# pola-rs/polars

Measured on AMD Instinct MI355X. Metric: rows/sec + achieved HBM GB/s, TPC-H Q1/Q3 SF100, 1/2/4/8 GPU vs CPU, higher is better.
Workload: dtype f64; 1 GPU; tpch_q1_sf100; rows_per_gpu=600000000, algorithmic_bytes_per_gpu_step=25200000000, parallelism=single GPU

## Files before the change

include/polars_amd.h:

```cpp
#ifndef POLARS_AMD_H
#define POLARS_AMD_H

#include <stddef.h>
#include <stdint.h>

#ifdef __cplusplus
extern "C" {
#endif

#define PLX_ABI_MAJOR 0
#define PLX_ABI_MINOR 1

#define PLX_OK 0
#define PLX_ERR_INVALID 1
#define PLX_ERR_HIP 2
#define PLX_ERR_UNSUPPORTED 3
#define PLX_ERR_OOM 4
#define PLX_ERR_SHAPE 5
#define PLX_ERR_NOT_FOUND 6
#define PLX_ERR_CANCELLED 7

typedef enum plx_dtype {
  PLX_BOOL = 0,
  PLX_I8 = 1,
// ... 181 lines not shown
  PLX_AE_IS_NOT_NULL = 9,
  PLX_AE_FILL_NULL = 10,
  PLX_AE_TERNARY = 11,
  PLX_AE_BITMAP_LOOKUP = 12,
  PLX_AE_TEMPORAL = 13
} plx_aexpr_kind;

typedef enum plx_operator {
  PLX_OP_EQ = 0, PLX_OP_NE = 1, PLX_OP_LT = 2, PLX_OP_LE = 3, PLX_OP_GT = 4, PLX_OP_GE = 5,
  PLX_OP_PLUS = 6, PLX_OP_MINUS = 7, PLX_OP_MULTIPLY = 8, PLX_OP_TRUE_DIVIDE = 9,
  PLX_OP_FLOOR_DIVIDE = 10, PLX_OP_MODULUS = 11, PLX_OP_AND = 12, PLX_OP_OR = 13, PLX_OP_XOR = 14
} plx_operator;

typedef struct plx_aexpr {
  int32_t kind;
  int32_t op;
  int32_t lhs;
  int32_t rhs;
  int32_t dtype;
  int32_t is_null;
  plx_scalar lit;
  const char* name;
  int32_t cond;
} plx_aexpr;

typedef enum plx_ir_kind {
  PLX_IR_SCAN = 0,
  PLX_IR_FILTER = 1,
  PLX_IR_SELECT = 2,
  PLX_IR_HSTACK = 3,
  PLX_IR_GROUPBY = 4,
  PLX_IR_JOIN = 5,
  PLX_IR_SORT = 6,
  PLX_IR_SLICE = 7
} plx_ir_kind;

typedef enum plx_join_order {
  PLX_JOIN_ORDER_NONE = 0,
  PLX_JOIN_ORDER_LEFT = 1,
  PLX_JOIN_ORDER_RIGHT = 2,
  PLX_JOIN_ORDER_LEFT_RIGHT = 3,
  PLX_JOIN_ORDER_RIGHT_LEFT = 4
} plx_join_order;

typedef struct plx_ir {
  int32_t kind;
  int32_t input;
  int32_t input_right;
  int32_t predicate;
  plx_frame frame;
  const int32_t* exprs;
  int32_t n_exprs;
  const int32_t* keys;
  int32_t n_keys;
  const int32_t* keys_right;
  int32_t n_keys_right;
  int32_t how;
  int32_t maintain_order;
  const char* suffix;
  const uint8_t* sort_descending;
  const uint8_t* sort_nulls_last;
  int64_t slice_offset;
  int64_t slice_len;
  int32_t coalesce;
} plx_ir;

#define PLX_PLAN_NO_FUSION 1u
#define PLX_PLAN_NO_PARTITION 4u
#define PLX_PLAN_NO_DIRECT_JOIN 2u

int plx_execute_plan(const plx_ir* ir, int32_t n_ir, const plx_aexpr* exprs, int32_t n_exprs, int32_t root,
                     uint32_t flags, plx_frame* out);
int plx_describe_fusion(const plx_ir* ir, int32_t n_ir, const plx_aexpr* exprs, int32_t n_exprs, int32_t root, int32_t* fusable,
                        int32_t* static_shape_id, char* why_not, size_t why_cap);
int plx_debug_program_json(const plx_ir* ir, int32_t n_ir, const plx_aexpr* exprs, int32_t n_exprs, int32_t root, char* buf, size_t cap);
int plx_jit_selftest(const plx_ir* ir, int32_t n_ir, const plx_aexpr* exprs, int32_t n_exprs, int32_t root);
int plx_jit_stats(int32_t* compiled, double* compile_ms);
int plx_jit_set_min_rows(int64_t min_rows);
const char* plx_last_plan_description(void);
const char* plx_last_plan_encodings(void);
int32_t plx_last_scan_tile_rows(void);
int32_t plx_wide_tiles_choice(int32_t compiled, int32_t knob_on, int64_t n_rows, int32_t n_inputs, const int32_t* dtypes, const int32_t* nullable, const uint64_t* values,
                              const uint64_t* validity);

int plx_datagen_lineitem_q1(int64_t n_rows, uint64_t seed, plx_column* out_cols);
int plx_datagen_lineitem_q1_host(int64_t row0, int64_t n, uint64_t seed, int64_t* shipdate, uint8_t* returnflag, uint8_t* linestatus,
                                 int64_t* quantity, double* extendedprice, double* discount, double* tax);

int plx_datagen_orders_lineitem(int64_t n_orders, uint64_t seed, plx_column* out_orders, plx_column* out_lineitem);
int plx_datagen_orders_lineitem_host(int64_t order0, int64_t n, int64_t n_orders_total, uint64_t seed, int64_t* orderkey, int64_t* custkey,
                                     int64_t* orderdate, uint32_t* n_lines, int64_t line_cap, int64_t* l_orderkey, double* l_extendedprice,
                                     double* l_discount, int64_t* l_shipdate, int64_t* n_lines_out);
int plx_datagen_customer(int64_t n_customers, uint64_t seed, plx_column* out_cols);
int plx_datagen_customer_host(int64_t row0, int64_t n, uint64_t seed, int64_t* custkey, uint8_t* segment);
int plx_datagen_uniform(int32_t dtype, int64_t n_rows, uint64_t seed, uint32_t stream, int64_t lo, int64_t hi, double scale, plx_column* out);
int plx_datagen_uniform_host(int32_t dtype, int64_t row0, int64_t n, uint64_t seed, uint32_t stream, int64_t lo, int64_t hi, double scale, void* out);
int plx_datagen_zipf(int64_t n_rows, uint64_t seed, uint32_t stream, uint64_t x0_q62, int64_t n_keys, plx_column* out);
int plx_datagen_zipf_host(int64_t row0, int64_t n, uint64_t seed, uint32_t stream, uint64_t x0_q62, int64_t n_keys, int64_t* out);

typedef uint64_t plx_strdict;
int plx_strview_dict_encode(const void* views, const uint8_t* validity, int64_t bit_offset, int64_t n, const void* const* data_buffers, const int64_t* data_sizes,
                            int32_t n_data_buffers, plx_column* out_codes, plx_strdict* out_dict);
int plx_strview_dict_encode_device(plx_column views_u64_pairs, plx_column data_u8, plx_column* out_codes, plx_strdict* out_dict);
int plx_strview_stamp_nulls(plx_column views_u64_pairs, plx_column valid_bool);
int plx_strview_groupby(plx_column views_u64_pairs, plx_column value, plx_column* out_codes, plx_strdict* out_dict, plx_column* out_sum, plx_column* out_count, plx_column* out_len);
#define PLX_STR_MATCH_MAX_PATTERN 64
typedef enum plx_str_match_kind { PLX_STR_STARTS_WITH = 0, PLX_STR_ENDS_WITH = 1, PLX_STR_CONTAINS = 2 } plx_str_match_kind;
int plx_strdict_match(plx_strdict dict, int32_t kind, const uint8_t* pattern, int64_t pattern_len, plx_column* out_bool);
int plx_strview_match(plx_column views_u64_pairs, plx_column data_u8, int32_t kind, const uint8_t* pattern, int64_t pattern_len, plx_column* out_bool);
int plx_strview_match_host(const void* views, const uint8_t* data, int64_t data_len, int64_t n, int32_t kind, const uint8_t* pattern, int64_t pattern_len,
                           uint64_t* out_bits, uint64_t* out_valid);
int plx_bitmap_lookup(plx_column codes, plx_column lut_bool, plx_column* out_bool);
int plx_strdict_info(plx_strdict dict, int64_t* n_strings, int64_t* total_bytes);

typedef enum plx_time_unit { PLX_UNIT_DATE = 0, PLX_UNIT_MS = 1, PLX_UNIT_US = 2, PLX_UNIT_NS = 3 } plx_time_unit;
typedef enum plx_temporal_part_kind {
  PLX_PART_YEAR = 0, PLX_PART_MONTH = 1, PLX_PART_DAY = 2, PLX_PART_QUARTER = 3, PLX_PART_WEEKDAY = 4, PLX_PART_ORDINAL_DAY = 5,
  PLX_PART_HOUR = 6, PLX_PART_MINUTE = 7, PLX_PART_SECOND = 8, PLX_PART_DATE = 9
} plx_temporal_part_kind;
int plx_temporal_part(plx_column col, int part, int unit, plx_column* out);
int plx_temporal_part_host(const void* values, int unit, int part, int64_t n, void* out);

int plx_strdict_to_host(plx_strdict dict, int64_t* offsets, uint8_t* bytes);
int plx_strdict_free(plx_strdict dict);
int plx_datagen_id_views(int64_t n_rows, uint64_t seed, uint32_t stream, int64_t lo, int64_t hi, plx_column* out_views);
int plx_datagen_long_id_views(int64_t n_rows, uint64_t seed, uint32_t stream, int64_t lo, int64_t hi, plx_column* out_views, plx_column* out_data);

typedef uint64_t plx_parquet;
int plx_parquet_open(const char* path, plx_parquet* out);
int plx_parquet_close(plx_parquet file);
int plx_parquet_shape(plx_parquet file, int64_t* num_rows, int32_t* num_row_groups, int32_t* num_columns);
int plx_parquet_column_info(plx_parquet file, int32_t column, const char** name, int32_t* dtype, int32_t* logical, int32_t* nullable);
int plx_parquet_column_timezone(plx_parquet file, int32_t column, const char** timezone);
int plx_parquet_row_group_info(plx_parquet file, int32_t row_group, int64_t* num_rows, int64_t* compressed_bytes);
int plx_parquet_chunk_info(plx_parquet file, int32_t row_group, int32_t column, int32_t* codec, uint32_t* encodings, int64_t* compressed_bytes,
                           int64_t* uncompressed_bytes, int32_t* has_min_max, plx_scalar* min, plx_scalar* max, int64_t* null_count);
int plx_parquet_read(plx_parquet file, const int32_t* row_groups, int32_t n_row_groups, const int32_t* columns, int32_t n_columns, plx_frame* out);
int plx_parquet_categories(plx_parquet file, int32_t column, int64_t* n_strings, int64_t* total_bytes);
int plx_parquet_categories_to_host(plx_parquet file, int32_t column, int64_t* offsets, uint8_t* bytes);
int plx_parquet_column_strdict(plx_parquet file, int32_t column, plx_strdict* out);

typedef uint64_t plx_ipc;
int plx_ipc_open(const char* path, plx_ipc* out);
int plx_ipc_close(plx_ipc file);
int plx_ipc_shape(plx_ipc file, int64_t* num_rows, int32_t* num_batches, int32_t* num_columns);
int plx_ipc_column_info(plx_ipc file, int32_t column, const char** name, int32_t* dtype, int32_t* logical, int32_t* nullable);
int plx_ipc_column_timezone(plx_ipc file, int32_t column, const char** timezone);
int plx_ipc_batch_info(plx_ipc file, int32_t batch, int64_t* num_rows, int64_t* body_bytes, int32_t* compressed);
int plx_ipc_read(plx_ipc file, const int32_t* batches, int32_t n_batches, const int32_t* columns, int32_t n_columns, plx_frame* out);
int plx_ipc_read_string_views(plx_ipc file, const int32_t* batches, int32_t n_batches, int32_t column, plx_column* out_views, plx_column* out_data);
int plx_ipc_categories(plx_ipc file, int32_t column, int64_t* n_strings, int64_t* total_bytes);
int plx_ipc_categories_to_host(plx_ipc file, int32_t column, int64_t* offsets, uint8_t* bytes);
int plx_ipc_column_strdict(plx_ipc file, int32_t column, plx_strdict* out);

typedef uint64_t plx_comm;
int plx_comm_unique_id(uint8_t* out_128_bytes);
int plx_comm_init(const uint8_t* unique_id_128_bytes, int32_t rank, int32_t world_size, plx_comm* out);
int plx_comm_info(plx_comm comm, int32_t* rank, int32_t* world_size);
int plx_comm_free(plx_comm comm);
int plx_exchange_by_key(plx_comm comm, plx_frame frame, const char* key, uint64_t seed, plx_frame* out, uint64_t* rows_sent, uint64_t* bytes_sent);
int plx_allgather_frame(plx_comm comm, plx_frame frame, plx_frame* out);

typedef struct plx_profile_record {
  char name[48];
  double start_us;
  double end_us;
// ... 33 lines not shown
```

polars_amd/_ffi.py:

```python
from __future__ import annotations

import ctypes as C
import os
import threading
from typing import Optional

os.environ.setdefault("GPU_MAX_HW_QUEUES", "8")

_HERE = os.path.dirname(os.path.abspath(__file__))
LIB_PATH = os.path.join(_HERE, "libpolars_amd.so")

BOOL, I8, I16, I32, I64, U8, U16, U32, U64, F32, F64 = range(11)
EQ, NE, LT, LE, GT, GE = range(6)
ADD, SUB, MUL, TRUE_DIV, FLOOR_DIV, MOD = range(6)
AND, OR, XOR = range(3)
AGG_SUM, AGG_MEAN, AGG_MIN, AGG_MAX, AGG_COUNT, AGG_LEN, AGG_FIRST, AGG_VAR, AGG_STD = range(9)
AGG_QUANTILE = 9
QUANTILE_NEAREST, QUANTILE_LOWER, QUANTILE_HIGHER, QUANTILE_MIDPOINT, QUANTILE_LINEAR = range(5)
QUANTILE_INTERPOLATIONS = {"nearest": QUANTILE_NEAREST, "lower": QUANTILE_LOWER, "higher": QUANTILE_HIGHER, "midpoint": QUANTILE_MIDPOINT, "linear": QUANTILE_LINEAR}
JOIN_INNER, JOIN_LEFT, JOIN_SEMI, JOIN_ANTI, JOIN_FULL, JOIN_RIGHT = range(6)
JOIN_COALESCE_DEFAULT, JOIN_COALESCE, JOIN_KEEP_BOTH = range(3)
JOIN_ORDER_NONE, JOIN_ORDER_LEFT, JOIN_ORDER_RIGHT, JOIN_ORDER_LEFT_RIGHT, JOIN_ORDER_RIGHT_LEFT = range(5)
AE_COLUMN, AE_LITERAL, AE_BINARY, AE_CAST, AE_AGG, AE_LEN, AE_ALIAS, AE_NOT, AE_IS_NULL, AE_IS_NOT_NULL, AE_FILL_NULL, AE_TERNARY, AE_BITMAP_LOOKUP, AE_TEMPORAL = range(14)
STR_STARTS_WITH, STR_ENDS_WITH, STR_CONTAINS = range(3)
# ... 120 lines not shown
    "plx_parquet_shape": (C.c_int, [C.c_uint64, _i64p, _i32p, _i32p]),
    "plx_parquet_column_info": (C.c_int, [C.c_uint64, C.c_int32, C.POINTER(C.c_char_p), _i32p, _i32p, _i32p]),
    "plx_parquet_column_timezone": (C.c_int, [C.c_uint64, C.c_int32, C.POINTER(C.c_char_p)]),
    "plx_parquet_row_group_info": (C.c_int, [C.c_uint64, C.c_int32, _i64p, _i64p]),
    "plx_parquet_chunk_info": (C.c_int, [C.c_uint64, C.c_int32, C.c_int32, _i32p, C.POINTER(C.c_uint32), _i64p, _i64p, _i32p, C.POINTER(Scalar), C.POINTER(Scalar), _i64p]),
    "plx_parquet_read": (C.c_int, [C.c_uint64, _i32p, C.c_int32, _i32p, C.c_int32, _u64p]),
    "plx_parquet_categories": (C.c_int, [C.c_uint64, C.c_int32, _i64p, _i64p]),
    "plx_parquet_categories_to_host": (C.c_int, [C.c_uint64, C.c_int32, C.c_void_p, C.c_void_p]),
    "plx_parquet_column_strdict": (C.c_int, [C.c_uint64, C.c_int32, _u64p]),
    "plx_ipc_open": (C.c_int, [C.c_char_p, _u64p]),
    "plx_ipc_close": (C.c_int, [C.c_uint64]),
    "plx_ipc_shape": (C.c_int, [C.c_uint64, _i64p, _i32p, _i32p]),
    "plx_ipc_column_info": (C.c_int, [C.c_uint64, C.c_int32, C.POINTER(C.c_char_p), _i32p, _i32p, _i32p]),
    "plx_ipc_column_timezone": (C.c_int, [C.c_uint64, C.c_int32, C.POINTER(C.c_char_p)]),
    "plx_ipc_batch_info": (C.c_int, [C.c_uint64, C.c_int32, _i64p, _i64p, _i32p]),
    "plx_ipc_read": (C.c_int, [C.c_uint64, _i32p, C.c_int32, _i32p, C.c_int32, _u64p]),
    "plx_ipc_read_string_views": (C.c_int, [C.c_uint64, _i32p, C.c_int32, C.c_int32, _u64p, _u64p]),
    "plx_ipc_categories": (C.c_int, [C.c_uint64, C.c_int32, _i64p, _i64p]),
    "plx_ipc_categories_to_host": (C.c_int, [C.c_uint64, C.c_int32, C.c_void_p, C.c_void_p]),
    "plx_ipc_column_strdict": (C.c_int, [C.c_uint64, C.c_int32, _u64p]),
    "plx_comm_unique_id": (C.c_int, [C.c_void_p]),
    "plx_comm_init": (C.c_int, [C.c_void_p, C.c_int32, C.c_int32, _u64p]),
    "plx_comm_info": (C.c_int, [C.c_uint64, C.POINTER(C.c_int32), C.POINTER(C.c_int32)]),
    "plx_comm_free": (C.c_int, [C.c_uint64]),
    "plx_exchange_by_key": (C.c_int, [C.c_uint64, C.c_uint64, C.c_char_p, C.c_uint64, _u64p, _u64p, _u64p]),
    "plx_allgather_frame": (C.c_int, [C.c_uint64, C.c_uint64, _u64p]),
    "plx_column_import_arrow": (C.c_int, [C.POINTER(ArrowArray), C.POINTER(ArrowSchema), _u64p]),
    "plx_column_import_series": (C.c_int, [C.POINTER(SeriesExport), _u64p]),
    "plx_column_export_arrow": (C.c_int, [C.c_uint64, C.POINTER(ArrowArray), C.POINTER(ArrowSchema)]),
    "plx_column_export_series": (C.c_int, [C.c_uint64, C.c_char_p, C.POINTER(SeriesExport)]),
    "plx_column_to_host": (C.c_int, [C.c_uint64, C.c_void_p, C.c_void_p, _i32p]),
    "plx_column_copy_to_device": (C.c_int, [C.c_uint64, C.c_void_p, C.c_void_p]),
    "plx_column_info": (C.c_int, [C.c_uint64, _i32p, _i64p, _i64p]),
    "plx_column_device_ptrs": (C.c_int, [C.c_uint64, C.POINTER(C.c_void_p), C.POINTER(C.c_void_p)]),
    "plx_column_retain": (C.c_int, [C.c_uint64]),
    "plx_column_free": (C.c_int, [C.c_uint64]),
    "plx_cmp": (C.c_int, [C.c_int, C.c_uint64, C.c_uint64, _u64p]),
    "plx_cmp_scalar": (C.c_int, [C.c_int, C.c_uint64, Scalar, _u64p]),
    "plx_bitmap_binop": (C.c_int, [C.c_int, C.c_uint64, C.c_uint64, _u64p]),
    "plx_bitmap_not": (C.c_int, [C.c_uint64, _u64p]),
    "plx_arith": (C.c_int, [C.c_int, C.c_uint64, C.c_uint64, _u64p]),
    "plx_arith_scalar": (C.c_int, [C.c_int, C.c_uint64, Scalar, C.c_int, _u64p]),
    "plx_cast": (C.c_int, [C.c_uint64, C.c_int, _u64p]),
    "plx_if_then_else": (C.c_int, [C.c_uint64, C.c_uint64, C.c_uint64, _u64p]),
    "plx_filter": (C.c_int, [C.c_uint64, C.c_uint64, _u64p]),
    "plx_gather": (C.c_int, [C.c_uint64, C.c_uint64, _u64p]),
    "plx_reduce": (C.c_int, [C.c_int, C.c_uint64, C.POINTER(Scalar), _i32p, _i32p]),
    "plx_reduce_var": (C.c_int, [C.c_uint64, C.c_int32, C.c_int32, C.POINTER(Scalar), _i32p, _i32p]),
    "plx_groupby_agg": (C.c_int, [_u64p, C.c_int32, _u64p, _i32p, C.c_int32, C.c_int32, _u64p, _u64p]),
    "plx_groupby_agg_ddof": (C.c_int, [_u64p, C.c_int32, _u64p, _i32p, C.c_int32, C.c_int32, _i32p, _u64p, _u64p]),
    "plx_reduce_quantile": (C.c_int, [C.c_uint64, C.c_double, C.c_int32, C.POINTER(Scalar), _i32p, _i32p]),
    "plx_groupby_agg_params": (C.c_int, [_u64p, C.c_int32, _u64p, _i32p, C.c_int32, C.c_int32, _i32p, C.POINTER(C.c_double), _i32p, _u64p, _u64p]),
    "plx_join_indices": (C.c_int, [C.c_int, C.c_uint64, C.c_uint64, _u64p, _u64p]),
    "plx_datagen_lineitem_q1": (C.c_int, [C.c_int64, C.c_uint64, _u64p]),
    "plx_datagen_lineitem_q1_host": (C.c_int, [C.c_int64, C.c_int64, C.c_uint64, C.c_void_p, C.c_void_p, C.c_void_p, C.c_void_p, C.c_void_p, C.c_void_p, C.c_void_p]),
    "plx_datagen_orders_lineitem": (C.c_int, [C.c_int64, C.c_uint64, _u64p, _u64p]),
    "plx_datagen_orders_lineitem_host": (C.c_int, [C.c_int64, C.c_int64, C.c_int64, C.c_uint64, C.c_void_p, C.c_void_p, C.c_void_p, C.c_void_p, C.c_int64,
                                                   C.c_void_p, C.c_void_p, C.c_void_p, C.c_void_p, _i64p]),
    "plx_datagen_uniform": (C.c_int, [C.c_int32, C.c_int64, C.c_uint64, C.c_uint32, C.c_int64, C.c_int64, C.c_double, _u64p]),
    "plx_datagen_customer": (C.c_int, [C.c_int64, C.c_uint64, _u64p]),
    "plx_datagen_customer_host": (C.c_int, [C.c_int64, C.c_int64, C.c_uint64, C.c_void_p, C.c_void_p]),
    "plx_datagen_uniform_host": (C.c_int, [C.c_int32, C.c_int64, C.c_int64, C.c_uint64, C.c_uint32, C.c_int64, C.c_int64, C.c_double, C.c_void_p]),
    "plx_datagen_zipf": (C.c_int, [C.c_int64, C.c_uint64, C.c_uint32, C.c_uint64, C.c_int64, _u64p]),
    "plx_datagen_zipf_host": (C.c_int, [C.c_int64, C.c_int64, C.c_uint64, C.c_uint32, C.c_uint64, C.c_int64, C.c_void_p]),
    "plx_debug_program_json": (C.c_int, [C.POINTER(IR), C.c_int32, C.POINTER(AExpr), C.c_int32, C.c_int32, C.c_char_p, C.c_size_t]),
    "plx_sort_indices": (C.c_int, [_u64p, C.c_int32, C.POINTER(C.c_uint8), C.POINTER(C.c_uint8), C.c_int64, _u64p]),
    "plx_hash_partition": (C.c_int, [C.c_uint64, C.c_int32, C.c_uint64, _u64p, _i64p]),
    "plx_frame_new": (C.c_int, [C.POINTER(C.c_char_p), _u64p, C.c_int32, _u64p]),
    "plx_frame_free": (C.c_int, [C.c_uint64]),
    "plx_frame_concat": (C.c_int, [_u64p, C.c_int32, _u64p]),
    "plx_frame_shape": (C.c_int, [C.c_uint64, _i64p, _i32p]),
    "plx_frame_column": (C.c_int, [C.c_uint64, C.c_int32, C.POINTER(C.c_char_p), _u64p]),
    "plx_frame_dtypes": (C.c_int, [C.c_uint64, _i32p]),
    "plx_frame_to_host": (C.c_int, [C.c_uint64, C.POINTER(C.c_void_p), C.POINTER(C.c_void_p), _i32p]),
    "plx_execute_plan": (C.c_int, [C.POINTER(IR), C.c_int32, C.POINTER(AExpr), C.c_int32, C.c_int32, C.c_uint32, _u64p]),
    "plx_describe_fusion": (C.c_int, [C.POINTER(IR), C.c_int32, C.POINTER(AExpr), C.c_int32, C.c_int32, _i32p, _i32p, C.c_char_p, C.c_size_t]),
    "plx_jit_selftest": (C.c_int, [C.POINTER(IR), C.c_int32, C.POINTER(AExpr), C.c_int32, C.c_int32]),
    "plx_jit_stats": (C.c_int, [_i32p, C.POINTER(C.c_double)]),
    "plx_jit_set_min_rows": (C.c_int, [C.c_int64]),
    "plx_last_plan_description": (C.c_char_p, []),
    "plx_last_plan_encodings": (C.c_char_p, []),
    "plx_last_scan_tile_rows": (C.c_int32, []),
    "plx_wide_tiles_choice": (C.c_int32, [C.c_int32, C.c_int32, C.c_int64, C.c_int32, C.POINTER(C.c_int32), C.POINTER(C.c_int32), C.POINTER(C.c_uint64), C.POINTER(C.c_uint64)]),
    "plx_profile_enable": (C.c_int, [C.c_int]),
    "plx_profile_fetch": (C.c_int, [C.POINTER(ProfileRecord), C.c_int32, _i32p]),
    "plx_profile_clear": (C.c_int, []),
}

_lib: Optional[C.CDLL] = None


def lib() -> C.CDLL:
    global _lib
    if _lib is None:
        if not os.path.exists(LIB_PATH):
            raise ImportError(
                f"{LIB_PATH} is missing: build the HIP extension first "
                "(python -c 'import __graft_entry__ as g; g.build()' or make -C polars_amd/csrc). "
                "There is no CPU fallback in polars_amd.")
        l = C.CDLL(LIB_PATH, mode=C.RTLD_GLOBAL)
        for name, (res, args) in SIGNATURES.items():
            fn = getattr(l, name)
            fn.restype = res
            fn.argtypes = args
        _lib = l
    return _lib


def check(status: int) -> None:
    if status != 0:
        msg = lib().plx_last_error().decode("utf-8", "replace")
        if status == ERR_UNSUPPORTED:
            raise UnsupportedError(status, msg)
        raise PlxError(status, msg)


_initialised = False


def init(device: Optional[int] = None) -> None:
    global _initialised
    if device is None:
        device = int(os.environ.get("LOCAL_RANK", "0"))
    check(lib().plx_init(device))
    _initialised = True


def ensure_init() -> None:
    if not _initialised:
        init()


_tls = threading.local()


def set_plan_note(note) -> None:
    _tls.plan_note = note


def last_plan() -> str:
    note = getattr(_tls, "plan_note", None)
    return note if note is not None else lib().plx_last_plan_description().decode()


def last_plan_encodings() -> str:
    return lib().plx_last_plan_encodings().decode()


def last_scan_tile_rows() -> int:
    return int(lib().plx_last_scan_tile_rows())


def wide_tiles_choice(compiled, knob_on, n_rows, dtypes, nullable, values, validity) -> int:
    n = len(dtypes)
    return int(lib().plx_wide_tiles_choice(int(bool(compiled)), int(bool(knob_on)), int(n_rows), n, (C.c_int32 * n)(*[int(d) for d in dtypes]),
                                           (C.c_int32 * n)(*[int(bool(x)) for x in nullable]), (C.c_uint64 * n)(*[int(v) for v in values]), (C.c_uint64 * n)(*[int(v) for v in validity])))


def jit_set_min_rows(min_rows: int) -> None:
    check(lib().plx_jit_set_min_rows(int(min_rows)))


def encoded_set_decimal_min_rows(min_rows: int) -> None:
    check(lib().plx_encoded_set_decimal_min_rows(int(min_rows)))


def encoded_decimal_min_rows() -> int:
    return int(lib().plx_encoded_decimal_min_rows())


def jit_stats():
    n, ms = C.c_int32(), C.c_double()
    check(lib().plx_jit_stats(C.byref(n), C.byref(ms)))
    return n.value, ms.value
```

polars_amd/csrc/abi.cpp:

```cpp
#include <cstdio>
#include <cstring>
#include <memory>
#include <mutex>

#include "core.hpp"
#include "datagen_device.hpp"
#include "encoded_inputs.hpp"
#include "engine.hpp"
#include "fused_shapes.hpp"
#include "jit.hpp"
#include "join.hpp"
#include "kernels.hpp"
#include "kernels_fused.hpp"
#include "ops.hpp"
#include "scan.hpp"
#include "sort.hpp"
#include "strmatch.hpp"
#include "temporal.hpp"

namespace plx {
void init_device(int ordinal);
void clear_handles();
const std::string& last_error_ref();
namespace comm {
void unique_id(uint8_t* out128);
uint64_t init(const uint8_t* id128, int rank, int ws);
void destroy(uint64_t h);
void info(uint64_t h, int* rank, int* ws);
FramePtr exchange_by_key(uint64_t h, const FramePtr& in, const std::string& key, uint64_t seed, uint64_t* rows_sent, uint64_t* bytes_sent);
FramePtr allgather_frame(uint64_t h, const FramePtr& in);
}
}

using namespace plx;

#define PLX_TRY try {
#define PLX_CATCH                                                                   \
  }                                                                                 \
  catch (const plx::Error& e) { plx::set_last_error(e.msg); return e.code; }        \
  catch (const std::bad_alloc&) { plx::set_last_error("host out of memory"); return PLX_ERR_OOM; } \
  catch (const std::exception& e) { plx::set_last_error(std::string("PANIC: ") + e.what()); return PLX_ERR_INVALID; } \
  catch (...) { plx::set_last_error("PANIC"); return PLX_ERR_INVALID; }              \
  return PLX_OK;

static thread_local std::string t_plan_desc;
static thread_local std::string t_plan_encoded;

extern "C" {

uint32_t plx_version(void) { return ((uint32_t)PLX_ABI_MAJOR << 16) | (uint32_t)PLX_ABI_MINOR; }
const char* plx_last_error(void) { return plx::last_error_ref().c_str(); }

int plx_init(int device_ordinal) { PLX_TRY init_device(device_ordinal); PLX_CATCH }
int plx_shutdown(void) {
  PLX_TRY
  clear_handles();
  pool_trim();
  PLX_CATCH
}
int plx_set_stream(void* hip_stream) { PLX_TRY device(); set_thread_stream((hipStream_t)hip_stream); PLX_CATCH }
int plx_synchronize(void) { PLX_TRY PLX_HIP(hipStreamSynchronize(stream())); PLX_CATCH }
int plx_set_cancel(int flag) { PLX_TRY device().cancel.store(flag); PLX_CATCH }
int plx_device_info(char* name_out, size_t name_cap, int32_t* cu_count, uint64_t* hbm_bytes) {
  PLX_TRY
  Device& d = device();
  if (name_out && name_cap) snprintf(name_out, name_cap, "%s", d.name.c_str());
  if (cu_count) *cu_count = d.cu_count;
  if (hbm_bytes) *hbm_bytes = d.hbm_bytes;
  PLX_CATCH
}
int plx_memory_stats(uint64_t* in_use, uint64_t* high_water) { PLX_TRY pool_stats(in_use, high_water); PLX_CATCH }
int plx_memory_trim(void) { PLX_TRY pool_trim(); PLX_CATCH }
int plx_memory_reserve(uint64_t bytes) { PLX_TRY device(); pool_reserve((size_t)bytes); PLX_CATCH }

int plx_column_from_host(plx_dtype dtype, const void* values, const uint8_t* validity, int64_t bit_offset, int64_t len, plx_column* out) {
  PLX_TRY
  PLX_REQUIRE(out, PLX_ERR_INVALID, "null out pointer");
  PLX_REQUIRE(values || len == 0, PLX_ERR_INVALID, "null values pointer");
  *out = register_column(column_from_host(dtype, values, validity, bit_offset, len));
  PLX_CATCH
}
int plx_column_from_device(plx_dtype dtype, void* dev_values, void* dev_validity, int64_t len, plx_column* out) {
  PLX_TRY
  device();
  PLX_REQUIRE(out && (dev_values || len == 0), PLX_ERR_INVALID, "null pointer");
  PLX_REQUIRE(dtype >= PLX_BOOL && dtype <= PLX_F64 && len >= 0, PLX_ERR_INVALID, "column_from_device: bad dtype or length");
  const uintptr_t value_align = dtype == PLX_BOOL ? 8 : (uintptr_t)dtype_width(dtype);
  PLX_REQUIRE(((uintptr_t)dev_values % value_align) == 0, PLX_ERR_INVALID,
              std::string("column_from_device: the values pointer of a ") + dtype_name(dtype) + " column must be a multiple of " + std::to_string(value_align));
  PLX_REQUIRE(((uintptr_t)dev_validity % 8) == 0, PLX_ERR_INVALID, "column_from_device: the validity pointer must be a multiple of 8 (validity is read as 64-bit words)");
  auto c = std::make_shared<Column>();
// ... 821 lines not shown
  }
  if (n_lines_out) *n_lines_out = at;
  PLX_CATCH
}
int plx_datagen_customer(int64_t n_customers, uint64_t seed, plx_column* out_cols) {
  PLX_TRY
  PLX_REQUIRE(n_customers >= 0 && out_cols, PLX_ERR_INVALID, "datagen: bad arguments");
  ColumnPtr k = make_column(PLX_I64, n_customers, false), sgm = make_column(PLX_U8, n_customers, false);
  k->null_count = 0; sgm->null_count = 0;
  k::datagen_customer(n_customers, seed, k->values->as<int64_t>(), sgm->values->as<uint8_t>());
  out_cols[0] = register_column(k); out_cols[1] = register_column(sgm);
  PLX_CATCH
}
int plx_datagen_customer_host(int64_t row0, int64_t n, uint64_t seed, int64_t* custkey, uint8_t* segment) {
  PLX_TRY
  PLX_REQUIRE(row0 >= 0 && n >= 0, PLX_ERR_INVALID, "datagen: bad arguments");
  for (int64_t j = 0; j < n; j++) {
    if (custkey) custkey[j] = row0 + j + 1;
    if (segment) segment[j] = datagen::customer_segment(seed, (uint64_t)(row0 + j + 1));
  }
  PLX_CATCH
}
int plx_datagen_uniform(int32_t dtype, int64_t n_rows, uint64_t seed, uint32_t stream_id, int64_t lo, int64_t hi, double scale, plx_column* out) {
  PLX_TRY
  PLX_REQUIRE(n_rows >= 0 && out && hi > lo && stream_id < 8, PLX_ERR_INVALID, "datagen: bad arguments");
  PLX_REQUIRE(dtype == PLX_I64 || dtype == PLX_U32 || dtype == PLX_F64, PLX_ERR_UNSUPPORTED, "datagen_uniform: dtype must be Int64, UInt32 or Float64");
  ColumnPtr c = make_column(dtype, n_rows, false); c->null_count = 0;
  k::datagen_uniform(dtype, n_rows, seed, stream_id, lo, hi, scale, c->values->ptr);
  *out = register_column(c);
  PLX_CATCH
}
int plx_datagen_uniform_host(int32_t dtype, int64_t row0, int64_t n, uint64_t seed, uint32_t stream_id, int64_t lo, int64_t hi, double scale, void* out) {
  PLX_TRY
  PLX_REQUIRE(row0 >= 0 && n >= 0 && (out || n == 0) && hi > lo && stream_id < 8, PLX_ERR_INVALID, "datagen: bad arguments");
  PLX_REQUIRE(dtype == PLX_I64 || dtype == PLX_U32 || dtype == PLX_F64, PLX_ERR_UNSUPPORTED, "datagen_uniform: dtype must be Int64, UInt32 or Float64");
  for (int64_t j = 0; j < n; j++) {
    const int64_t v = datagen::uniform_value(seed, stream_id, (uint64_t)(row0 + j), lo, hi);
    if (dtype == PLX_I64) reinterpret_cast<int64_t*>(out)[j] = v;
    else if (dtype == PLX_U32) reinterpret_cast<uint32_t*>(out)[j] = (uint32_t)v;
    else reinterpret_cast<double*>(out)[j] = (double)v * scale;
  }
  PLX_CATCH
}

int plx_datagen_zipf(int64_t n_rows, uint64_t seed, uint32_t stream_id, uint64_t x0_q62, int64_t n_keys, plx_column* out) {
  PLX_TRY
  PLX_REQUIRE(n_rows >= 0 && out && n_keys > 0 && stream_id < 8 && x0_q62 > 0 && x0_q62 < (1ull << 62), PLX_ERR_INVALID, "datagen_zipf: bad arguments");
  ColumnPtr c = make_column(PLX_I64, n_rows, false); c->null_count = 0;
  k::datagen_zipf(n_rows, seed, stream_id, x0_q62, n_keys, c->values->as<int64_t>());
  *out = register_column(c);
  PLX_CATCH
}
int plx_datagen_zipf_host(int64_t row0, int64_t n, uint64_t seed, uint32_t stream_id, uint64_t x0_q62, int64_t n_keys, int64_t* out) {
  PLX_TRY
  PLX_REQUIRE(row0 >= 0 && n >= 0 && (out || n == 0) && n_keys > 0 && stream_id < 8 && x0_q62 > 0 && x0_q62 < (1ull << 62), PLX_ERR_INVALID, "datagen_zipf: bad arguments");
  for (int64_t j = 0; j < n; j++) out[j] = datagen::zipf_value(seed, stream_id, (uint64_t)(row0 + j), x0_q62, n_keys);
  PLX_CATCH
}

int plx_execute_plan(const plx_ir* ir, int32_t n_ir, const plx_aexpr* exprs, int32_t n_exprs, int32_t root, uint32_t flags, plx_frame* out) {
  PLX_TRY
  PLX_REQUIRE(out, PLX_ERR_INVALID, "null out pointer");
  engine::Plan p = engine::import_plan(ir, n_ir, exprs, n_exprs, flags);
  FramePtr f = engine::execute(p, root);
  t_plan_desc = p.desc;
  t_plan_encoded = p.encoded;
  *out = register_frame(f);
  PLX_CATCH
}
const char* plx_last_plan_description(void) { return t_plan_desc.c_str(); }
const char* plx_last_plan_encodings(void) { return t_plan_encoded.c_str(); }
int32_t plx_last_scan_tile_rows(void) { return k::last_scan_tile_rows(); }
int32_t plx_wide_tiles_choice(int32_t compiled, int32_t knob_on, int64_t n_rows, int32_t n_inputs, const int32_t* dtypes, const int32_t* nullable, const uint64_t* values,
                              const uint64_t* validity) {
  if (n_inputs < 0 || n_inputs > fused::kMaxInputs || (n_inputs && (!dtypes || !nullable || !values || !validity))) return -1;
  fused::Shape sh{}; fused::Args args{};
  sh.n_inputs = (uint8_t)n_inputs; sh.pred = fused::kNone; sh.key = fused::kNone;
  args.n_rows = n_rows;
  for (int i = 0; i < n_inputs; i++) {
    sh.in_dtype[i] = (uint8_t)dtypes[i]; sh.in_nullable[i] = (uint8_t)(nullable[i] != 0);
    args.in[i].values = (const void*)(uintptr_t)values[i]; args.in[i].validity = (const uint64_t*)(uintptr_t)validity[i];
  }
  return k::wide_tiles_choice(sh, args, compiled != 0, knob_on != 0) ? 1 : 0;
}

int plx_debug_program_json(const plx_ir* ir, int32_t n_ir, const plx_aexpr* exprs, int32_t n_exprs, int32_t root, char* buf, size_t cap) {
  PLX_TRY
  PLX_REQUIRE(buf && cap > 0, PLX_ERR_INVALID, "null buffer");
  engine::Plan p = engine::import_plan(ir, n_ir, exprs, n_exprs, 0);
  std::string json, why;
  if (!engine::dump_program_json(p, root, &json, &why)) fail(PLX_ERR_UNSUPPORTED, "not a fusable pipeline: " + why);
  PLX_REQUIRE(json.size() + 1 <= cap, PLX_ERR_INVALID, "buffer too small for the program dump (" + std::to_string(json.size() + 1) + " bytes)");
  memcpy(buf, json.c_str(), json.size() + 1);
  PLX_CATCH
}

int plx_describe_fusion(const plx_ir* ir, int32_t n_ir, const plx_aexpr* exprs, int32_t n_exprs, int32_t root, int32_t* fusable, int32_t* static_shape_id,
                        char* why_not, size_t why_cap) {
  PLX_TRY
  engine::Plan p = engine::import_plan(ir, n_ir, exprs, n_exprs, 0);
  auto dump = [](const fused::Shape& sh) {
    std::string d = "inputs=" + std::to_string(sh.n_inputs) + " pred=" + std::to_string(sh.pred) + " key=" + std::to_string(sh.key) + " ops=[";
    for (int i = 0; i < sh.n_ops; i++) d += "(" + std::to_string(sh.ops[i].code) + "," + std::to_string(sh.ops[i].dst) + "," + std::to_string(sh.ops[i].a) + "," + std::to_string(sh.ops[i].b) + "," + std::to_string(sh.ops[i].c) + ")";
    d += "] aggs=[";
    for (int i = 0; i < sh.n_aggs; i++) d += "(" + std::to_string(sh.aggs[i].kind) + "," + std::to_string(sh.aggs[i].src) + ")";
    d += "] in_dtype=[";
    for (int i = 0; i < sh.n_inputs; i++) d += std::to_string(sh.in_dtype[i]) + (sh.in_nullable[i] ? "?" : "") + ",";
    d += "]";
    if (sh.n_keys) { d += " keys=["; for (int i = 0; i < sh.n_keys; i++) d += std::to_string(sh.keys[i]) + ","; d += "]"; }
    return d;
  };
  std::string why;
  int sid = -1;
  bool ok;
  PLX_REQUIRE(root >= 0 && root < (int)p.ir.size(), PLX_ERR_INVALID, "bad root");
  const engine::IRN& rn = p.ir[root];
  if (rn.kind == PLX_IR_GROUPBY && rn.input >= 0 && p.ir[rn.input].kind == PLX_IR_JOIN) {
    std::vector<fused::Shape> shapes;
    ok = engine::describe_join_fusion(p, root, &shapes, &why);
    if (ok) {
      sid = fused::find_static_shape(shapes[2]);
      t_plan_desc = dump(shapes[0]);
      for (size_t i = 1; i < shapes.size(); i++) t_plan_desc += "\n" + dump(shapes[i]);
    }
  } else {
    fused::Shape sh{};
    ok = engine::describe_fusion(p, root, &sh, &sid, &why);
    if (ok) t_plan_desc = dump(sh);
  }
  if (fusable) *fusable = ok ? 1 : 0;
  if (static_shape_id) *static_shape_id = sid;
  if (why_not && why_cap) snprintf(why_not, why_cap, "%s", why.c_str());
  PLX_CATCH
}

int plx_jit_selftest(const plx_ir* ir, int32_t n_ir, const plx_aexpr* exprs, int32_t n_exprs, int32_t root) {
  PLX_TRY
  engine::Plan p = engine::import_plan(ir, n_ir, exprs, n_exprs, 0);
  PLX_REQUIRE(root >= 0 && root < (int)p.ir.size(), PLX_ERR_INVALID, "bad root");
  const engine::IRN& rn = p.ir[root];
  std::string why;
  std::vector<std::pair<fused::Shape, jit::Sink>> jobs;
  if (rn.kind == PLX_IR_GROUPBY && rn.input >= 0 && p.ir[rn.input].kind == PLX_IR_JOIN) {
    std::vector<fused::Shape> shapes;
    PLX_REQUIRE(engine::describe_join_fusion(p, root, &shapes, &why), PLX_ERR_UNSUPPORTED, "not fusable: " + why);
    jobs = {{shapes[0], jit::REGAGG}, {shapes[1], jit::JOIN_BUILD}, {shapes[1], jit::DIRECT_BUILD}, {shapes[2], jit::PROBE_AGG}, {shapes[2], jit::DIRECT_PROBE}};
    for (size_t i = 3; i + 1 < shapes.size(); i++) jobs.push_back({shapes[i], jit::BITMAP_BUILD});
    for (uint32_t tiles : {2u, 4u}) jobs.push_back({shapes.back(), jit::part3_scatter_sink(fused::kP2Direct, tiles, fused::kPackRowid, false)});
  } else if (rn.kind == PLX_IR_FILTER) {
    fused::Shape sh{};
    PLX_REQUIRE(engine::describe_filter_fusion(p, root, &sh, &why), PLX_ERR_UNSUPPORTED, "not fusable: " + why);
    jobs = {{sh, jit::BALLOT}};
  } else {
    fused::Shape sh{}; int sid = -1;
    PLX_REQUIRE(engine::describe_fusion(p, root, &sh, &sid, &why), PLX_ERR_UNSUPPORTED, "not fusable: " + why);
    if (rn.kind == PLX_IR_SELECT) jobs = {{sh, jit::REGAGG}};
    else jobs = {{sh, jit::LDSAGG}, {sh, jit::DENSE}, {sh, jit::HASH}, {sh, jit::PART_COUNT}, {sh, jit::PART_SCATTER}, {sh, jit::PART_AGG},
                  {sh, jit::PART2_SCATTER_HASH}, {sh, jit::PART2_SCATTER_DIRECT}, {sh, jit::PART2_AGG_HASH}, {sh, jit::PART2_AGG_DIRECT},
                  {sh, jit::PART2_SCATTER_HASH_T2}, {sh, jit::PART2_SCATTER_DIRECT_T2}};
    if (rn.kind != PLX_IR_SELECT && sh.n_keys < 2) {
      for (uint32_t mode = 0; mode < 2; mode++) {
        const uint32_t best = fused::best_static_pack(sh, mode);
        for (uint32_t pack = 0; pack <= best; pack++) {
          if (pack == fused::kPackNarrow && fused::rec_layout2(sh, mode, fused::kPackNarrow).rec_words == fused::rec_layout2(sh, mode, fused::kPackNone).rec_words) continue;
          for (uint32_t tiles : {1u, 2u, 3u, 4u}) { jobs.push_back({sh, jit::part3_scatter_sink(mode, tiles, pack, false)}); jobs.push_back({sh, jit::part3_scatter_sink(mode, tiles, pack, true)}); }
          jobs.push_back({sh, jit::part3_agg_sink(mode, pack)});
        }
      }
      for (uint32_t mode = 0; mode < 2; mode++) {
        if (!fused::pair_pack_ok(sh, mode)) continue;
        for (uint32_t tiles : {1u, 2u, 3u, 4u}) { if (mode == fused::kP2Hash && tiles > 3) continue; jobs.push_back({sh, jit::part3_scatter_sink(mode, tiles, fused::kPackPair, false)}); jobs.push_back({sh, jit::part3_scatter_sink(mode, tiles, fused::kPackPair, true)}); }
        jobs.push_back({sh, jit::part3_agg_sink(mode, fused::kPackPair)});
      }
      if (fused::pairv_pack_ok(sh, fused::kP2Hash)) {
        for (uint32_t tiles : {1u, 2u, 3u}) { jobs.push_back({sh, jit::part3_scatter_sink(fused::kP2Hash, tiles, fused::kPackPairV, false)}); jobs.push_back({sh, jit::part3_scatter_sink(fused::kP2Hash, tiles, fused::kPackPairV, true)}); }
        jobs.push_back({sh, jit::part3_agg_sink(fused::kP2Hash, fused::kPackPairV)});
      }
    }
    if (sh.n_keys >= 2) {
      jobs = {{sh, jit::WIDE}};
      for (uint32_t pack = 0; pack <= std::min<uint32_t>(fused::best_static_pack(sh, fused::kP2Hash), fused::kPackNarrow); pack++) {
        for (uint32_t tiles : {1u, 2u, 3u}) jobs.push_back({sh, jit::part3_scatter_sink(fused::kP2Hash, tiles, pack, false)});
        jobs.push_back({sh, jit::part3_agg_sink(fused::kP2Hash, pack)});
      }
    }
  }
  {
    std::vector<std::pair<fused::Shape, jit::Sink>> forms;
    fused::Args aligned{}; aligned.n_rows = fused::kWideTileRows;
    for (auto& j : jobs) {
      const bool wide = k::wide_tiles_choice(j.first, aligned, true, true);
      if (j.second == jit::REGAGG && wide) forms.push_back({j.first, jit::REGAGG_WIDE});
      if (j.second == jit::LDSAGG && wide) forms.push_back({j.first, jit::LDSAGG_WIDE});
    }
    jobs.insert(jobs.end(), forms.begin(), forms.end());
  }
  for (auto& j : jobs) {
    const std::string log = jit::selftest(j.first, j.second);
    if (!log.empty()) fail(PLX_ERR_INVALID, "jit selftest failed: " + log.substr(0, 4000));
  }
  PLX_CATCH
}
int plx_jit_set_min_rows(int64_t min_rows) { PLX_TRY jit::set_min_rows(min_rows); PLX_CATCH }
int plx_jit_stats(int32_t* compiled, double* compile_ms) {
  PLX_TRY
  int c = 0; double ms = 0;
  jit::stats(&c, &ms);
  if (compiled) *compiled = c;
  if (compile_ms) *compile_ms = ms;
  PLX_CATCH
}

extern "C++" {
namespace {
struct StrDict { Buf views, data, offsets, bytes; int64_t n = 0; uint64_t total = 0; bool materialised = false; };
std::mutex g_strdict_mu;
std::vector<std::unique_ptr<StrDict>> g_strdicts;
StrDict& get_strdict(uint64_t h) {
  std::lock_guard<std::mutex> lk(g_strdict_mu);
  if (h == 0 || h > g_strdicts.size() || !g_strdicts[h - 1]) fail(PLX_ERR_INVALID, "invalid string dictionary handle");
  return *g_strdicts[h - 1];
}
uint64_t register_strdict(std::unique_ptr<StrDict> d) { std::lock_guard<std::mutex> lk(g_strdict_mu); g_strdicts.push_back(std::move(d)); return (uint64_t)g_strdicts.size(); }
void materialise(StrDict& d) {
  if (d.materialised) return;
  k::strdict_materialise(d.views->as<uint64_t>(), d.data ? d.data->as<uint8_t>() : nullptr, d.n, &d.offsets, &d.bytes, &d.total);
  d.materialised = true;
}
void encode_on_device(const uint64_t* views, const ColumnPtr& validity_holder, Buf data, Buf buf_base, int64_t n, plx_column* out_codes, plx_strdict* out_dict, bool from_stamps = false) {
  Buf codes, dviews, svalid;
  int64_t nd = 0, snulls = 0;
  k::strview_dict_encode(views, validity_holder ? validity_holder->valid_words() : nullptr, data ? data->as<uint8_t>() : nullptr, buf_base ? buf_base->as<uint64_t>() : nullptr, n, &codes, &dviews, &nd,
                         from_stamps && !validity_holder ? &svalid : nullptr, &snulls);
  auto c = std::make_shared<Column>();
  c->dtype = PLX_U32; c->len = n; c->values = codes;
  if (validity_holder && validity_holder->validity) c->validity = validity_holder->validity;
  else if (snulls > 0) { c->validity = svalid; c->null_count = snulls; }
  else c->null_count = 0;
  if (nd > 0) { c->range_state = 1; c->range_min = 0; c->range_max = nd - 1; c->range_trusted = true; }
  auto d = std::make_unique<StrDict>();
  d->views = dviews; d->data = data; d->n = nd;
  *out_codes = register_column(c);
  *out_dict = register_strdict(std::move(d));
}
}
namespace plx {
void strview_encode_device(const uint64_t* views, const ColumnPtr& validity_holder, Buf data, int64_t n, plx_column* out_codes, plx_strdict* out_dict) {
  Buf bb = dev_alloc_zero(8);
  encode_on_device(views, validity_holder, data, bb, n, out_codes, out_dict);
}
void strview_encode_device_bases(const uint64_t* views, const ColumnPtr& validity_holder, Buf data, Buf buf_base, int64_t n, plx_column* out_codes, plx_strdict* out_dict) {
  encode_on_device(views, validity_holder, data, buf_base, n, out_codes, out_dict);
}
}
}

int plx_strview_dict_encode(const void* views, const uint8_t* validity, int64_t bit_offset, int64_t n, const void* const* data_buffers, const int64_t* data_sizes,
                            int32_t n_data_buffers, plx_column* out_codes, plx_strdict* out_dict) {
  PLX_TRY
  PLX_REQUIRE(out_codes && out_dict && n >= 0 && (views || n == 0) && n_data_buffers >= 0 && (n_data_buffers == 0 || (data_buffers && data_sizes)), PLX_ERR_INVALID, "strview_dict_encode: bad arguments");
  device();
  Buf dv = dev_alloc((size_t)std::max<int64_t>(n, 1) * 16);
  if (n) h2d_sync_pinned(dv->ptr, views, (size_t)n * 16);
  ColumnPtr vh;
  if (validity) {
    std::vector<uint8_t> zeros((size_t)n);
    vh = column_from_host(PLX_U8, zeros.data(), validity, bit_offset, n);
  }
  uint64_t total = 0;
  std::vector<uint64_t> base((size_t)std::max(n_data_buffers, 1), 0);
  for (int i = 0; i < n_data_buffers; i++) { base[i] = total; total += (uint64_t)data_sizes[i]; }
  Buf data = dev_alloc((size_t)total + 64), bb = dev_alloc(sizeof(uint64_t) * base.size());
  for (int i = 0; i < n_data_buffers; i++) {
    if (!data_sizes[i]) continue;
    if ((uint64_t)data_sizes[i] >= ((uint64_t)32 << 20)) h2d_sync_pinned((uint8_t*)data->ptr + base[i], data_buffers[i], (size_t)data_sizes[i]);
    else h2d_async((uint8_t*)data->ptr + base[i], data_buffers[i], (size_t)data_sizes[i]);
// ... 248 lines not shown
```

polars_amd/csrc/fused_device.hpp:

```cpp
#pragma once
#include "decimal.hpp"
#include "dev.hpp"
#include "fused.hpp"
#include "fused_shapes.hpp"
#include "kconfig.hpp"
#include "temporal.hpp"

namespace plx {
namespace k {

using namespace dev;
using namespace fused;

typedef unsigned long long u64x16 __attribute__((ext_vector_type(16)));
typedef unsigned int u32x16 __attribute__((ext_vector_type(16)));

struct RegFile {
  uint64_t v[kRows][kSlots];
  uint32_t valid[kSlots];
  __device__ __forceinline__ uint64_t get(int r, int s) const { return v[r][s]; }
  __device__ __forceinline__ uint32_t getv(int s) const { return valid[s]; }
  __device__ __forceinline__ void set(int r, int s, uint64_t x) { v[r][s] = x; }
  __device__ __forceinline__ void setv(int s, uint32_t m) { valid[s] = m; }
};
struct LdsRegFile {
  unsigned long long* vals;
  unsigned int* vbits;
  int lane;
  __device__ __forceinline__ uint64_t get(int r, int s) const { return vals[(s * kRows + r) * 64 + lane]; }
  __device__ __forceinline__ uint32_t getv(int s) const { return vbits[s * 64 + lane]; }
  __device__ __forceinline__ void set(int r, int s, uint64_t x) { vals[(s * kRows + r) * 64 + lane] = x; }
  __device__ __forceinline__ void setv(int s, uint32_t m) { vbits[s * 64 + lane] = m; }
};
__host__ __device__ constexpr unsigned lds_regfile_bytes_per_wave(unsigned slots) { return slots * (kRows * 64 * 8 + 64 * 4); }

__device__ __forceinline__ int dtype_width_dev(int dt) {
  switch (dt) {
    case PLX_I8: case PLX_U8: return 1;
    case PLX_I16: case PLX_U16: return 2;
    case PLX_I32: case PLX_U32: case PLX_F32: return 4;
    default: return 8;
  }
}
__device__ __forceinline__ double as_f(uint64_t x) { return __longlong_as_double((long long)x); }
__device__ __forceinline__ uint64_t as_u(double x) { return (uint64_t)__double_as_longlong(x); }

template <class T, bool FULL>
__device__ __forceinline__ void load2(const void* base_ptr, int64_t row0, int64_t n, uint64_t out[kRows]) {
  const T* p = reinterpret_cast<const T*>(base_ptr);
  if constexpr (FULL) {
    Pack<T, kRows> x = load_pack<T, kRows>(p + row0);
#pragma unroll
    for (int r = 0; r < kRows; r++) {
      if constexpr (is_fp<T>::value) out[r] = as_u((double)x.v[r]);
      else out[r] = (uint64_t)(long long)x.v[r];
    }
  } else {
#pragma unroll
    for (int r = 0; r < kRows; r++) {
      int64_t i = row0 + r; if (i > n - 1) i = n - 1;
      T x = p[i];
      if constexpr (is_fp<T>::value) out[r] = as_u((double)x);
      else out[r] = (uint64_t)(long long)x;
    }
  }
}

template <bool FULL>
__device__ __forceinline__ void load_input(const Input& in, int dtype, int64_t row0, int64_t n, uint64_t out[kRows], uint32_t& vbits, bool may_be_null = true) {
  switch (dtype) {
    case PLX_I64: case PLX_U64: case PLX_F64: load2<uint64_t, FULL>(in.values, row0, n, out); break;
    case PLX_I32: load2<int32_t, FULL>(in.values, row0, n, out); break;
    case PLX_U32: load2<uint32_t, FULL>(in.values, row0, n, out); break;
    case PLX_I16: load2<int16_t, FULL>(in.values, row0, n, out); break;
    case PLX_U16: load2<uint16_t, FULL>(in.values, row0, n, out); break;
    case PLX_I8: load2<int8_t, FULL>(in.values, row0, n, out); break;
    case PLX_U8: load2<uint8_t, FULL>(in.values, row0, n, out); break;
    case PLX_BOOL: {
      int64_t i = row0; if (!FULL && i > n - 1) i = n - 1;
      uint64_t w = reinterpret_cast<const uint64_t*>(in.values)[i >> 6] >> (i & 63);
      out[0] = w & 1; out[1] = (w >> 1) & 1;
    } break;
    default: out[0] = out[1] = 0; break;
  }
  vbits = (1u << kRows) - 1;
  if (may_be_null && in.validity) {
// ... 290 lines not shown
    for (int pc = 0; pc < sh.n_ops; pc++) exec_op<FULL, ND, TRUST_NULLABLE>(sh.ops[pc], sh, args, pc, row0, rf);
  } else {
    Prefetched pf;
    pf.bits0 = 0; pf.bits1 = 0; pf.vword = 0;
    prefetch_inputs<FULL>(dsh, args, row0, pf);
    store_prefetched<FULL>(dsh, args, row0, pf, rf);
    const int first = dsh.n_inputs < kPrefetch ? dsh.n_inputs : kPrefetch;
    for (int pc = first; pc < dsh.n_ops; pc++) exec_op<FULL>(dsh.ops[pc], dsh, args, pc, row0, rf);
  }
}

__host__ __device__ constexpr int leading_loads(const Shape& s) {
  int n = 0;
  while (n < s.n_ops && s.ops[n].code == OP_LOAD) n++;
  return n;
}
__host__ __device__ constexpr int shape_row_bytes(const Shape& s) {
  int b = 0;
  for (int i = 0; i < s.n_inputs; i++) {
    switch (s.in_dtype[i]) {
      case PLX_I8: case PLX_U8: b += 1; break;
      case PLX_I16: case PLX_U16: b += 2; break;
      case PLX_I32: case PLX_U32: case PLX_F32: b += 4; break;
      case PLX_BOOL: break;
      default: b += 8; break;
    }
  }
  return b;
}
__host__ __device__ constexpr bool narrow_rows(const Shape& s) { return s.n_inputs > 0 && shape_row_bytes(s) <= 16; }
__host__ __device__ constexpr int wide_dtype_bytes(int dt) {
  switch (dt) {
    case PLX_I8: case PLX_U8: return 1;
    case PLX_I16: case PLX_U16: return 2;
    case PLX_I32: case PLX_U32: return 4;
    case PLX_I64: case PLX_U64: case PLX_F64: return 8;
    default: return 0;
  }
}
__host__ __device__ constexpr bool wide_tiles_shape(const Shape& s) {
  if (!narrow_rows(s)) return false;
  bool any_narrow = false;
  for (int i = 0; i < s.n_inputs; i++) {
    if (s.in_nullable[i] != 0 || wide_dtype_bytes(s.in_dtype[i]) == 0) return false;
    any_narrow = any_narrow || wide_dtype_bytes(s.in_dtype[i]) < 8;
  }
  if (!any_narrow) return false;
  for (int pc = 0; pc < s.n_ops; pc++) if (s.ops[pc].code == OP_LOAD && s.ops[pc].a >= s.n_inputs) return false;
  return true;
}
struct WideRaw { uint32_t w[kMaxInputs][2 * kWideRows]; };
template <class P>
__device__ __forceinline__ void wide_load(const Args& args, int64_t row0, WideRaw& raw) {
  constexpr Shape sh = P::shape();
#pragma unroll
  for (int i = 0; i < kMaxInputs; i++) {
    if (i < sh.n_inputs) {
      const int wb = wide_dtype_bytes(sh.in_dtype[i]);
      const unsigned char* p = reinterpret_cast<const unsigned char*>(args.in[i].values) + row0 * wb;
      if (wb == 1) {
        const uint2 x = *reinterpret_cast<const uint2*>(p);
        raw.w[i][0] = x.x; raw.w[i][1] = x.y;
      } else {
#pragma unroll
        for (int q = 0; q < wb / 2; q++) {
          const uint4 x = reinterpret_cast<const uint4*>(p)[q];
          raw.w[i][4 * q] = x.x; raw.w[i][4 * q + 1] = x.y; raw.w[i][4 * q + 2] = x.z; raw.w[i][4 * q + 3] = x.w;
        }
      }
    }
  }
}
__device__ __forceinline__ uint64_t wide_unpack(const uint32_t* w, int dt, int e) {
  switch (dt) {
    case PLX_I8: return (uint64_t)(long long)(int8_t)(w[e >> 2] >> ((e & 3) * 8));
    case PLX_U8: return (uint64_t)(uint8_t)(w[e >> 2] >> ((e & 3) * 8));
    case PLX_I16: return (uint64_t)(long long)(int16_t)(w[e >> 1] >> ((e & 1) * 16));
    case PLX_U16: return (uint64_t)(uint16_t)(w[e >> 1] >> ((e & 1) * 16));
    case PLX_I32: return (uint64_t)(long long)(int32_t)w[e];
    case PLX_U32: return (uint64_t)w[e];
    default: return (uint64_t)w[2 * e] | ((uint64_t)w[2 * e + 1] << 32);
  }
}
template <class P, int ND, class RF>
__device__ __forceinline__ void run_program_wide(const Args& args, const WideRaw& raw, int j, RF& rf) {
  constexpr Shape sh = P::shape();
#pragma unroll
  for (int pc = 0; pc < sh.n_ops; pc++) {
    const Op op = sh.ops[pc];
    if (op.code == OP_LOAD) {
#pragma unroll
      for (int r = 0; r < kRows; r++) rf.set(r, op.dst, wide_unpack(raw.w[op.a], sh.in_dtype[op.a], kRows * j + r));
      rf.setv(op.dst, (1u << kRows) - 1);
    } else {
      exec_op<true, ND, true>(op, sh, args, pc, 0, rf);
    }
  }
}

template <class P, class RF>
__device__ __forceinline__ void run_loads_full(const Args& args, int64_t row0, RF& rf) {
  constexpr Shape sh = P::shape();
  constexpr int nl = leading_loads(sh);
#pragma unroll
  for (int pc = 0; pc < nl; pc++) exec_op<true>(sh.ops[pc], sh, args, pc, row0, rf);
}
template <class P, class RF>
__device__ __forceinline__ void run_rest_full(const Args& args, int64_t row0, RF& rf) {
  constexpr Shape sh = P::shape();
  constexpr int nl = leading_loads(sh);
#pragma unroll
  for (int pc = nl; pc < sh.n_ops; pc++) exec_op<true>(sh.ops[pc], sh, args, pc, row0, rf);
}

template <class P, bool FULL, bool EARLY, class RF>
__device__ __forceinline__ void run_split(const Args& args, int64_t row0, RF& rf) {
  constexpr Shape sh = P::shape();
  constexpr ProgramSplit sp = split_program(sh);
#pragma unroll
  for (int pc = 0; pc < sh.n_ops; pc++)
    if (((sp.early >> pc) & 1u) == (EARLY ? 1u : 0u)) exec_op<FULL>(sh.ops[pc], sh, args, pc, row0, rf);
}

template <class P> struct RegFileOf { using type = RegFile; };
template <> struct RegFileOf<DynProg> { using type = LdsRegFile; };
template <class P>
__device__ __forceinline__ typename RegFileOf<P>::type make_regfile(const Args& args) {
  if constexpr (P::kStatic) { return RegFile{}; }
  else {
    extern __shared__ unsigned long long plx_dyn_lds[];
    const unsigned per_wave = lds_regfile_bytes_per_wave(args.rf_slots);
    unsigned char* base = reinterpret_cast<unsigned char*>(plx_dyn_lds) + args.rf_lds_offset + (threadIdx.x >> 6) * per_wave;
    LdsRegFile rf;
    rf.vals = reinterpret_cast<unsigned long long*>(base);
    rf.vbits = reinterpret_cast<unsigned int*>(base + (size_t)args.rf_slots * kRows * 64 * 8);
    rf.lane = lane_id();
    return rf;
  }
}

__device__ __forceinline__ uint64_t agg_combine(uint8_t kind, uint64_t x, uint64_t y) {
  switch (kind) {
    case AGG_SUM_F: return as_u(as_f(x) + as_f(y));
    case AGG_MIN_F: return as_u(min_ign<double>(as_f(x), as_f(y)));
    case AGG_MAX_F: return as_u(max_ign<double>(as_f(x), as_f(y)));
    case AGG_MIN_I: return (uint64_t)((long long)x < (long long)y ? (long long)x : (long long)y);
    case AGG_MAX_I: return (uint64_t)((long long)x > (long long)y ? (long long)x : (long long)y);
    case AGG_MIN_U: case AGG_FIRST_ROW: return x < y ? x : y;
    case AGG_MAX_U: return x > y ? x : y;
    default: return x + y;
  }
}
__device__ __forceinline__ uint64_t agg_identity_dev(uint8_t kind) {
  switch (kind) {
    case AGG_MIN_F: return 0x7ff0000000000000ull;
    case AGG_MAX_F: return 0xfff0000000000000ull;
    case AGG_MIN_I: return 0x7fffffffffffffffull;
    case AGG_MAX_I: return 0x8000000000000000ull;
    case AGG_MIN_U: case AGG_FIRST_ROW: return ~0ull;
    default: return 0ull;
  }
}
__device__ __forceinline__ uint64_t agg_row_value(uint8_t kind, uint64_t v, bool pass, bool valid, uint64_t row) {
  switch (kind) {
    case AGG_LEN: return pass ? 1ull : 0ull;
    case AGG_COUNT: return (pass && valid) ? 1ull : 0ull;
    case AGG_COUNT_ORD: { double f = as_f(v); return (pass && valid && f == f) ? 1ull : 0ull; }
    case AGG_FIRST_ROW: return pass ? row : ~0ull;
    case AGG_MIN_F: { double f = as_f(v); return (pass && valid && f == f) ? v : 0x7ff0000000000000ull; }
    case AGG_MAX_F: { double f = as_f(v); return (pass && valid && f == f) ? v : 0xfff0000000000000ull; }
    case AGG_SUM_F: case AGG_SUM_I: return (pass && valid) ? v : 0ull;
    default: return (pass && valid) ? v : agg_identity_dev(kind);
  }
}

// ... 90 lines not shown
```

polars_amd/csrc/fused_sinks.hpp:

```cpp
#pragma once
#include <type_traits>

#include "fused_device.hpp"

namespace plx {
namespace k {

struct RegAggSink {
  struct Params { unsigned long long* partials; };
  uint64_t acc[kMaxAggs];
  template <class S> __device__ __forceinline__ void init(const S& sh, const Params&) {
#pragma unroll
    for (int k = 0; k < kMaxAggs; k++) acc[k] = (k < sh.n_aggs) ? agg_identity_dev(sh.aggs[k].kind) : 0ull;
  }
  template <class S, class RF> __device__ __forceinline__ void consume(const S& sh, const RF& rf, const bool pass[kRows], int64_t row0, const Params&) {
#pragma unroll
    for (int r = 0; r < kRows; r++) {
#pragma unroll
      for (int k = 0; k < kMaxAggs; k++) {
        if (k < sh.n_aggs) {
          const Agg ag = sh.aggs[k];
          uint64_t v = rf.get(r, ag.src);
          bool valid = (rf.getv(ag.src) >> r) & 1;
          acc[k] = agg_combine(ag.kind, acc[k], agg_row_value(ag.kind, v, pass[r], valid, (uint64_t)(row0 + r)));
        }
      }
    }
  }
  template <class S> __device__ __forceinline__ void finish(const S& sh, const Params& p) {
    __shared__ uint64_t sh_acc[kBlock / 64][kMaxAggs];
    const int lane = lane_id(), wave = threadIdx.x >> 6;
#pragma unroll
    for (int k = 0; k < kMaxAggs; k++) {
      if (k < sh.n_aggs) {
        uint64_t x = acc[k];
#pragma unroll
        for (int m = 32; m >= 1; m >>= 1) x = agg_combine(sh.aggs[k].kind, x, shfl_xor_u64(x, m));
        if (lane == 0) sh_acc[wave][k] = x;
      }
    }
    __syncthreads();
    if ((int)threadIdx.x < sh.n_aggs) {
      const int k = threadIdx.x;
      uint64_t x = sh_acc[0][k];
      for (int w = 1; w < (int)(blockDim.x >> 6); w++) x = agg_combine(sh.aggs[k].kind, x, sh_acc[w][k]);
      p.partials[(size_t)blockIdx.x * kMaxAggs + k] = x;
    }
  }
};

struct LdsAggSink {
  struct Params {
    unsigned long long* partials;
    unsigned long long* global_acc;
    int n_groups;
    int copies;
    unsigned int* oob;
  };
  template <class S> __device__ __forceinline__ void init(const S& sh, const Params& p) {
    extern __shared__ unsigned long long lds_tbl[];
    const int cells = p.n_groups * sh.n_aggs;
    for (int i = threadIdx.x; i < cells * p.copies; i += blockDim.x) lds_tbl[i] = agg_identity_dev(sh.aggs[(i / p.copies) % sh.n_aggs].kind);
    __syncthreads();
  }
  template <class S, class RF> __device__ __forceinline__ void consume(const S& sh, const RF& rf, const bool pass[kRows], int64_t row0, const Params& p) {
    extern __shared__ unsigned long long lds_tbl[];
    const int copy = lane_id() & (p.copies - 1);
#pragma unroll
    for (int r = 0; r < kRows; r++) {
      if (!pass[r]) continue;
      const uint64_t gid64 = rf.get(r, sh.key);
      if (gid64 >= (uint64_t)p.n_groups) { if (p.oob) *p.oob = 1u; continue; }
      const uint32_t gid = (uint32_t)gid64;
      unsigned long long* cells = lds_tbl + (size_t)gid * sh.n_aggs * p.copies + copy;
#pragma unroll
      for (int k = 0; k < kMaxAggs; k++) {
        if (k < sh.n_aggs) {
          const Agg ag = sh.aggs[k];
          uint64_t v = rf.get(r, ag.src);
          bool valid = (rf.getv(ag.src) >> r) & 1;
          if ((ag.kind == AGG_SUM_F || ag.kind == AGG_SUM_I || ag.kind == AGG_COUNT) && !valid) continue;
          uint64_t x = agg_row_value(ag.kind, v, true, valid, (uint64_t)(row0 + r));
          lds_atomic_agg(ag.kind, cells + k * p.copies, x);
        }
      }
    }
  }
  template <class S> __device__ __forceinline__ void finish(const S& sh, const Params& p) {
    extern __shared__ unsigned long long lds_tbl[];
    __syncthreads();
    const int cells = p.n_groups * sh.n_aggs;
    for (int i = threadIdx.x; i < cells; i += blockDim.x) {
      const uint8_t kind = sh.aggs[i % sh.n_aggs].kind;
      uint64_t x = lds_tbl[(size_t)i * p.copies];
      for (int c = 1; c < p.copies; c++) x = agg_combine(kind, x, lds_tbl[(size_t)i * p.copies + c]);
      if (p.global_acc) { if (x != agg_identity_dev(kind) || kind == AGG_SUM_F) atomic_agg(kind, p.global_acc + i, x); }
      else p.partials[(size_t)blockIdx.x * cells + i] = x;
    }
  }
};

struct DenseAggSink {
  using Params = DenseTable;
  template <class S> __device__ __forceinline__ void init(const S&, const Params&) {}
  template <class S> __device__ __forceinline__ void finish(const S&, const Params&) {}
  template <class S, class RF> __device__ __forceinline__ void consume(const S& sh, const RF& rf, const bool pass[kRows], int64_t row0, const Params& p) {
#pragma unroll
    for (int r = 0; r < kRows; r++) {
      if (!pass[r]) continue;
      bool kvalid = (rf.getv(sh.key) >> r) & 1;
      int64_t g = kvalid ? ((int64_t)rf.get(r, sh.key) - p.key_min) : p.n_groups;
      if ((uint64_t)g > (uint64_t)p.n_groups || (kvalid && g == p.n_groups)) { if (p.oob) *p.oob = 1u; continue; }
      atomic_row(sh, rf, r, row0 + r, p.acc + (size_t)g * sh.n_aggs);
    }
  }
};

struct HashAggSink {
  using Params = HashTable;
  template <class S> __device__ __forceinline__ void init(const S&, const Params&) {}
  template <class S> __device__ __forceinline__ void finish(const S&, const Params&) {}
  __device__ __forceinline__ static int64_t find_slot(const Params& p, uint64_t key) {
    const uint64_t cap = 1ull << p.log2_cap;
    uint64_t slot = (key * 0x55fbfd6bfc5458e9ull) >> (64 - p.log2_cap);
    for (uint32_t probe = 0; probe < p.max_probe; probe++) {
      unsigned long long cur = p.keys[slot];
      if (cur == key) return (int64_t)slot;
      if (cur == kEmptyKey) {
        unsigned long long old = atomicCAS(&p.keys[slot], (unsigned long long)kEmptyKey, (unsigned long long)key);
        if (old == kEmptyKey || old == key) return (int64_t)slot;
      }
      slot = (slot + 1) & (cap - 1);
    }
    atomicExch(p.overflow, 1u);
    return -1;
  }
  static constexpr int kCombineRounds = 8;
  template <class S, class RF> __device__ __forceinline__ void consume_combined(const S& sh, const RF& rf, const bool pass[kRows], int64_t row0, const Params& p) {
    const uint64_t cap = 1ull << p.log2_cap;
    const int lane = lane_id();
#pragma unroll
    for (int r = 0; r < kRows; r++) {
      const bool kvalid = (rf.getv(sh.key) >> r) & 1;
      const uint64_t key = kvalid ? rf.get(r, sh.key) : 0ull;
      uint64_t xv[kMaxAggs];
#pragma unroll
      for (int k = 0; k < kMaxAggs; k++) {
        xv[k] = 0;
        if (k < sh.n_aggs) { const Agg ag = sh.aggs[k]; xv[k] = agg_row_value(ag.kind, rf.get(r, ag.src), true, (rf.getv(ag.src) >> r) & 1, (uint64_t)(row0 + r)); }
      }
      bool reached = false, keeps_total = false;
      uint64_t todo = ballot(pass[r]);
#pragma unroll 1
      for (int round = 0; round < kCombineRounds && todo; round++) {
        const int leader = (int)__builtin_ctzll(todo);
        const uint64_t lkey = shfl_u64(key, leader);
        const bool lvalid = __shfl((int)kvalid, leader, 64) != 0;
        const bool member = pass[r] && !reached && kvalid == lvalid && key == lkey;
        todo &= ~ballot(member);
#pragma unroll
        for (int k = 0; k < kMaxAggs; k++) {
          if (k < sh.n_aggs) {
            uint64_t x = member ? xv[k] : agg_identity_dev(sh.aggs[k].kind);
#pragma unroll
            for (int m = 32; m >= 1; m >>= 1) x = agg_combine(sh.aggs[k].kind, x, shfl_xor_u64(x, m));
            if (lane == leader) xv[k] = x;
          }
        }
        if (member) reached = true;
        if (lane == leader) keeps_total = true;
      }
      if (!pass[r] || (reached && !keeps_total)) continue;
      int64_t slot;
      if (!kvalid) { slot = (int64_t)cap; p.keys[cap] = 0; }
      else if (key == kEmptyKey) { slot = (int64_t)cap + 1; p.keys[cap + 1] = 0; }
      else slot = find_slot(p, key);
      if (slot < 0) continue;
#pragma unroll
      for (int k = 0; k < kMaxAggs; k++) {
        if (k < sh.n_aggs) {
          const uint8_t kind = sh.aggs[k].kind;
// ... 240 lines not shown
};

struct BitmapBuildSink {
  using Params = BitmapBuild;
  unsigned long long n = 0;
  template <class S> __device__ __forceinline__ void init(const S&, const Params&) { n = 0; }
  template <class S> __device__ __forceinline__ void finish(const S&, const Params& p) {
    const uint64_t w = wave_sum_u64(n);
    if (lane_id() == 0 && w) atomicAdd(p.count, (unsigned long long)w);
  }
  template <class S, class RF> __device__ __forceinline__ void consume(const S& sh, const RF& rf, const bool pass[kRows], int64_t, const Params& p) {
#pragma unroll
    for (int r = 0; r < kRows; r++) {
      if (!pass[r] || !((rf.getv(sh.key) >> r) & 1)) continue;
      const uint64_t idx = rf.get(r, sh.key) - (uint64_t)p.kmin;
      if (idx >= p.range) continue;
      n++;
      __hip_atomic_fetch_or(&p.bits[idx >> 6], 1ull << (idx & 63), __ATOMIC_RELAXED, __HIP_MEMORY_SCOPE_AGENT);
    }
  }
};

struct DirectHitsSink {
  using Params = DirectHits;
  template <class S> __device__ __forceinline__ void init(const S&, const Params&) {}
  template <class S> __device__ __forceinline__ void finish(const S&, const Params&) {}
  template <class S, class RF> __device__ __forceinline__ void consume(const S& sh, const RF& rf, const bool pass[kRows], int64_t row0, const Params& p) {
    bool hit[kRows];
#pragma unroll
    for (int r = 0; r < kRows; r++) {
      bool ok = pass[r] && ((rf.getv(sh.key) >> r) & 1);
      const uint64_t idx = rf.get(r, sh.key) - (uint64_t)p.t.kmin;
      ok = ok && idx < p.t.range;
      if (ok) ok = (p.t.bits[idx >> 6] >> (idx & 63)) & 1ull;
      hit[r] = ok;
    }
    const unsigned long long b0 = ballot(hit[0]), b1 = ballot(hit[1]);
    if (lane_id() == 0) {
      const int64_t t = row0 / kTileRows;
      *reinterpret_cast<ulonglong2*>(p.out.ballots + t * 2) = make_ulonglong2(b0, b1);
      p.out.counts[t] = (unsigned int)(popc64(b0) + popc64(b1));
    }
  }
};

template <class P, bool FULL>
__device__ __forceinline__ void direct_probe_tile(const Args& args, const DirectJoinTable& p, int64_t base, RegFile& rf) {
  constexpr Shape sh = P::shape();
  const int64_t row0 = base + (int64_t)lane_id() * kRows;
  run_split<P, FULL, true>(args, row0, rf);
  if (!(p.opts & kDirectLateLoads)) run_split<P, FULL, false>(args, row0, rf);
  bool hit[kRows], any = false;
  unsigned long long slot[kRows];
#pragma unroll
  for (int r = 0; r < kRows; r++) {
    bool ok = FULL || (row0 + r < args.n_rows);
    if (sh.pred != kNone) ok = ok && (rf.get(r, sh.pred) & 1) && ((rf.getv(sh.pred) >> r) & 1);
    ok = ok && ((rf.getv(sh.key) >> r) & 1);
    const uint64_t idx = rf.get(r, sh.key) - (uint64_t)p.kmin;
    ok = ok && idx < p.range;
    slot[r] = 0;
    if (ok) {
      const unsigned long long w = p.bits[idx >> 6];
      ok = (w >> (idx & 63)) & 1ull;
      if (ok) slot[r] = direct_slot(p, idx, w);
    }
    hit[r] = ok; any = any || ok;
  }
  if (any) {
    if (p.opts & kDirectLateLoads) run_split<P, FULL, false>(args, row0, rf);
#pragma unroll
    for (int r = 0; r < kRows; r++)
      if (hit[r]) atomic_row(sh, rf, r, row0 + r, p.acc + (size_t)slot[r] * sh.n_aggs);
  }
}

template <class P, class Sink>
__host__ __device__ constexpr bool late_probe() {
  if constexpr (P::kStatic && std::is_same<Sink, DirectProbeAggSink>::value) return split_program(P::shape()).any_late;
  else return false;
}
template <class P, class Sink>
__host__ __device__ constexpr bool trust_nullable() {
  if constexpr (P::kStatic && (std::is_same<Sink, LdsAggSink>::value || std::is_same<Sink, RegAggSink>::value)) return narrow_rows(P::shape());
  else return false;
}
template <class P, class Sink>
__host__ __device__ constexpr bool wide_tiles_form() {
  if constexpr (trust_nullable<P, Sink>()) return wide_tiles_shape(P::shape());
  else return false;
}
template <class P, class Sink, bool WIDE = false>
__device__ __forceinline__ void fused_scan_body(const Shape dsh, const Args args, const typename Sink::Params sp) {
  Sink sink;
  typename RegFileOf<P>::type rf = make_regfile<P>(args);
  const int64_t wave = ((int64_t)blockIdx.x * blockDim.x + threadIdx.x) >> 6;
  const int64_t nwaves = ((int64_t)gridDim.x * blockDim.x) >> 6;
  const int64_t ntiles = (args.n_rows + kTileRows - 1) / kTileRows;
  if constexpr (late_probe<P, Sink>()) {
    for (int64_t t = wave; t < ntiles; t += nwaves) {
      const int64_t base = t * kTileRows;
      if (base + kTileRows <= args.n_rows) direct_probe_tile<P, true>(args, sp, base, rf);
      else direct_probe_tile<P, false>(args, sp, base, rf);
    }
  } else if constexpr (P::kStatic) {
    constexpr Shape sh = P::shape();
    constexpr int ND = dict_count(sh);
    constexpr bool kTrust = trust_nullable<P, Sink>();
    if constexpr (ND > 0) { stage_dicts<ND>(args); __syncthreads(); }
    sink.init(sh, sp);
    int64_t first_tile = 0;
    if constexpr (WIDE) {
      static_assert(wide_tiles_form<P, Sink>(), "wide tiles: a compiled aggregate scan over narrow rows without nullable inputs");
      const int64_t nwide = args.n_rows / kWideTileRows;
      const int lane = lane_id();
      for (int64_t t = wave; t < nwide; t += nwaves) {
        const int64_t row0 = t * kWideTileRows + (int64_t)lane * kWideRows;
        WideRaw raw;
        wide_load<P>(args, row0, raw);
#pragma unroll
        for (int j = 0; j < kWideRows / kRows; j++) {
          run_program_wide<P, ND>(args, raw, j, rf);
          bool pass[kRows];
#pragma unroll
          for (int r = 0; r < kRows; r++) pass[r] = sh.pred == kNone || ((rf.get(r, sh.pred) & 1) && ((rf.getv(sh.pred) >> r) & 1));
          sink.consume(sh, rf, pass, row0 + kRows * j, sp);
        }
      }
      first_tile = nwide * (kWideTileRows / kTileRows);
    }
    for (int64_t t = first_tile + wave; t < ntiles; t += nwaves) {
      bool pass[kRows]; int64_t row0;
      tile_rows<P, ND, kTrust>(dsh, args, t, rf, pass, row0);
      sink.consume(sh, rf, pass, row0, sp);
    }
    sink.finish(sh, sp);
  } else {
    sink.init(dsh, sp);
    for (int64_t t = wave; t < ntiles; t += nwaves) {
      bool pass[kRows]; int64_t row0;
      tile_rows<P>(dsh, args, t, rf, pass, row0);
      sink.consume(dsh, rf, pass, row0, sp);
    }
    sink.finish(dsh, sp);
  }
}

template <class P, class Sink>
__global__ __launch_bounds__(kBlock) void fused_scan_kernel(Shape dsh, Args args, typename Sink::Params sp) {
  fused_scan_body<P, Sink>(dsh, args, sp);
}
template <class P, class Sink>
__global__ __launch_bounds__(kBlock) void fused_scan_wide_kernel(Shape dsh, Args args, typename Sink::Params sp) {
  fused_scan_body<P, Sink, true>(dsh, args, sp);
}

struct BallotSink {
  using Params = BallotOut;
  template <class S> __device__ __forceinline__ void init(const S&, const Params&) {}
  template <class S> __device__ __forceinline__ void finish(const S&, const Params&) {}
  template <class S, class RF> __device__ __forceinline__ void consume(const S&, const RF&, const bool pass[kRows], int64_t row0, const Params& p) {
    const unsigned long long b0 = ballot(pass[0]), b1 = ballot(pass[1]);
    if (lane_id() == 0) {
      const int64_t t = row0 / kTileRows;
      *reinterpret_cast<ulonglong2*>(p.ballots + t * 2) = make_ulonglong2(b0, b1);
      p.counts[t] = (unsigned int)(popc64(b0) + popc64(b1));
    }
  }
};

}
}
```

polars_amd/csrc/jit.cpp:

```cpp
#include "jit.hpp"

#include <dlfcn.h>
#include <sys/stat.h>
#include <unistd.h>
#include <hip/hip_runtime_api.h>
#include <hip/hiprtc.h>

#include <atomic>
#include <chrono>
#include <cstdlib>
#include <cstring>
#include <map>
#include <mutex>
#include <sstream>
#include <string>
#include <vector>

#include "core.hpp"
#include "kconfig.hpp"

namespace plx {
namespace jit {

using namespace fused;

namespace {
struct Entry { hipModule_t mod = nullptr; hipFunction_t fn = nullptr; bool failed = false; };
std::mutex g_mu;
std::map<std::string, Entry> g_cache;
int g_compiled = 0;
double g_ms = 0;

bool wide_tiles(Sink s) { return s == REGAGG_WIDE || s == LDSAGG_WIDE; }
const char* sink_type(Sink s) {
  static const char* n[] = {"RegAggSink", "LdsAggSink", "DenseAggSink", "HashAggSink", "WideAggSink", "JoinBuildSink", "ProbeAggSink", "DirectBuildSink", "DirectProbeAggSink", "BitmapBuildSink",
                            "part_count", "part_scatter", "part_agg", "part2_scatter_hash", "part2_scatter_direct", "part2_agg_hash", "part2_agg_direct", "part2_scatter_hash_t2", "part2_scatter_direct_t2"};
  if (s == REGAGG_WIDE) return "RegAggSink";
  if (s == LDSAGG_WIDE) return "LdsAggSink";
  if (s == PART3_AGG_PAIRV) return "part3_agg";
  if (s >= PART3_SCATTER_PAIRV && s < PART3_AGG_PAIRV) return "part3_scatter";
  if (s == PART3_AGG_PAIR || s == PART3_AGG_PAIR_DIRECT) return "part3_agg";
  if (s >= PART3_SCATTER_PAIR && s < PART3_AGG_PAIR) return "part3_scatter";
  if (s == BALLOT) return "BallotSink";
  if (s == DIRECT_HITS) return "DirectHitsSink";
  if (s >= PART3_AGG) return "part3_agg";
  if (s >= PART3_SCATTER) return "part3_scatter";
  return n[s];
}

std::string include_dir() {
  if (const char* e = getenv("PLX_JIT_INCLUDE")) return e;
  Dl_info info;
  if (dladdr((const void*)&stats, &info) && info.dli_fname) {
    std::string p = info.dli_fname;
    size_t k = p.rfind('/');
    return (k == std::string::npos ? std::string(".") : p.substr(0, k)) + "/csrc";
  }
  return "polars_amd/csrc";
}

std::string resource_include() {
  if (const char* e = getenv("PLX_JIT_CLANG_INCLUDE")) return e;
  const char* roots[] = {"/opt/rocm/lib/llvm/lib/clang", "/opt/rocm/llvm/lib/clang"};
  for (const char* r : roots) {
    for (int v = 30; v >= 14; v--) {
      const std::string p = std::string(r) + "/" + std::to_string(v) + "/include";
      if (FILE* f = fopen((p + "/stddef.h").c_str(), "r")) { fclose(f); return p; }
    }
  }
  return "/opt/rocm/lib/llvm/lib/clang/22/include";
}
std::vector<std::string> compile_options() {
  std::vector<std::string> o = {"--offload-arch=gfx950", "-O3", "-std=c++17", "-ffp-contract=off", "-munsafe-fp-atomics", "-Wno-pass-failed", "-ffreestanding",
                                "-I" + include_dir(), "-I/opt/rocm/include", "-I" + resource_include()};
  if (const char* e = getenv("PLX_JIT_DEFINES")) { std::istringstream is(e); std::string t; while (is >> t) if (t.compare(0, 2, "-D") == 0) o.push_back(t); }
  return o;
}

uint64_t fnv1a(const std::string& s, uint64_t h = 0xcbf29ce484222325ull) { for (unsigned char c : s) { h ^= c; h *= 0x100000001b3ull; } return h; }

std::string kernel_symbol(const Shape& sh, Sink sink) {
  std::string key((const char*)&sh, sizeof(Shape));
  key.push_back((char)sink);
  char out[96];
  snprintf(out, sizeof out, "plx_jit_%s_%d_%08x", sink_type(sink), (int)sink, (unsigned)(fnv1a(key) & 0xffffffffu));
  return out;
}

std::string source_for(const Shape& sh, Sink sink) {
  std::ostringstream o;
  const std::string sym = kernel_symbol(sh, sink);
  o << "#define plx_jit_kernel " << sym << "\n";
  o << ((sink == BALLOT || sink == DIRECT_HITS || wide_tiles(sink)) ? "#include \"fused_sinks.hpp\"\n" : sink >= PART3_SCATTER ? "#include \"partition3_device.hpp\"\n" : sink >= PART2_SCATTER_HASH ? "#include \"partition2_device.hpp\"\n" : sink >= PART_COUNT ? "#include \"partition_device.hpp\"\n" : "#include \"fused_sinks.hpp\"\n") << "namespace plx { namespace k {\n"
       "struct JitProg {\n  static constexpr bool kStatic = true; static constexpr int kId = -2;\n  static constexpr Shape shape() {\n    Shape s{};\n";
  o << "    s.n_inputs = " << (int)sh.n_inputs << "; s.n_ops = " << (int)sh.n_ops << "; s.n_aggs = " << (int)sh.n_aggs << "; s.pred = " << (int)sh.pred
    << "; s.key = " << (int)sh.key << "; s.n_keys = " << (int)sh.n_keys << ";\n";
  for (int i = 0; i < kMaxKeys; i++) o << "    s.keys[" << i << "] = " << (int)sh.keys[i] << ";\n";
  for (int i = 0; i < sh.n_inputs; i++) o << "    s.in_dtype[" << i << "] = " << (int)sh.in_dtype[i] << "; s.in_nullable[" << i << "] = " << (int)sh.in_nullable[i] << ";\n";
  for (int i = 0; i < sh.n_ops; i++)
    o << "    s.ops[" << i << "] = mkop(" << (int)sh.ops[i].code << ", " << (int)sh.ops[i].dst << ", " << (int)sh.ops[i].a << ", " << (int)sh.ops[i].b << ", " << (int)sh.ops[i].c << ");\n";
  for (int i = 0; i < sh.n_aggs; i++) o << "    s.aggs[" << i << "] = Agg{" << (int)sh.aggs[i].kind << ", " << (int)sh.aggs[i].src << "};\n";
  o << "    return s;\n  }\n};\n";
  switch (sink) {
    case PART_COUNT:
      o << "extern \"C\" __global__ __launch_bounds__(kBlock) void plx_jit_kernel(Shape dsh, Args args, uint32_t log2_parts, unsigned int* hist) {\n"
           "  part_count_body<JitProg>(dsh, args, log2_parts, hist);\n}\n}}\n";
      break;
    case PART_SCATTER:
      o << "extern \"C\" __global__ __launch_bounds__(kBlock) void plx_jit_kernel(Shape dsh, Args args, PartitionPlan pp, const unsigned long long* part_off, "
           "const unsigned long long* wg_prefix, unsigned long long* out) {\n  part_scatter_body<JitProg>(dsh, args, pp, part_off, wg_prefix, out);\n}\n}}\n";
      break;
    case PART_AGG:
      o << "extern \"C\" __global__ __launch_bounds__(kAggBlock) void plx_jit_kernel(Shape dsh, PartitionPlan pp, PartAggParams ap) {\n"
           "  constexpr Shape csh = JitProg::shape(); constexpr RecLayout cl = rec_layout(JitProg::shape());\n  part_agg_body(csh, cl, pp, ap);\n}\n}}\n";
      break;
    case PART2_SCATTER_HASH: case PART2_SCATTER_DIRECT: case PART2_SCATTER_HASH_T2: case PART2_SCATTER_DIRECT_T2:
      o << "extern \"C\" __global__ __launch_bounds__(kP2MaxBlock) void plx_jit_kernel(Shape dsh, Args args, PartPlan2 pp, ScatterParams2 sp) {\n"
           "  part2_scatter_body<JitProg, " << ((sink == PART2_SCATTER_DIRECT || sink == PART2_SCATTER_DIRECT_T2) ? 1 : 0) << ", "
        << ((sink == PART2_SCATTER_HASH_T2 || sink == PART2_SCATTER_DIRECT_T2) ? 2 : 1) << ">(dsh, args, pp, sp);\n}\n}}\n";
      break;
    case PART2_AGG_HASH: case PART2_AGG_DIRECT:
      o << "extern \"C\" __global__ __launch_bounds__(kP2AggBlock) void plx_jit_kernel(PartPlan2 pp, AggParams2 ap) {\n"
           "  constexpr Shape csh = JitProg::shape(); constexpr RecLayout2 cl = rec_layout2(JitProg::shape(), " << (sink == PART2_AGG_DIRECT ? 1 : 0) << "u);\n"
           "  part2_agg_body<Shape, " << (sink == PART2_AGG_DIRECT ? 1 : 0) << ", p2_agg_chunks_in_flight(cl.rec_words)>(csh, cl, pp, ap);\n}\n}}\n";
      break;
    default:
      if (wide_tiles(sink)) {
        o << "extern \"C\" __global__ __launch_bounds__(kBlock) void plx_jit_kernel(Shape dsh, Args args, " << sink_type(sink)
          << "::Params sp) {\n  fused_scan_body<JitProg, " << sink_type(sink) << ", true>(dsh, args, sp);\n}\n}}\n";
        break;
      }
      if (sink == PART3_AGG_PAIRV) {
        o << "extern \"C\" __global__ __launch_bounds__(kP2AggBlock) void plx_jit_kernel(PartPlan2 pp, AggParams2 ap) {\n"
             "  constexpr Shape csh = JitProg::shape(); constexpr RecLayout2 cl = rec_layout2(JitProg::shape(), 0u, " << fused::kPackPairV << "u);\n"
             "  part2_agg_body<Shape, 0, p2_agg_chunks_in_flight(cl.rec_words)>(csh, cl, pp, ap);\n}\n}}\n";
        break;
      }
      if (sink >= PART3_SCATTER_PAIRV && sink < PART3_AGG_PAIRV) {
        const int v = (int)sink - (int)PART3_SCATTER_PAIRV, tiles = 1 + (v & 3), hot = (v >> 2) & 1;
        o << "extern \"C\" __global__ __launch_bounds__(kP2MaxBlock) void plx_jit_kernel(Shape dsh, Args args, PartPlan2 pp, ScatterParams2 sp) {\n"
             "  part3_scatter_body<JitProg, 0, " << tiles << ", " << fused::kPackPairV << ", " << (hot ? "true" : "false") << ">(dsh, args, pp, sp);\n}\n}}\n";
        break;
      }
      if (sink == PART3_AGG_PAIR || sink == PART3_AGG_PAIR_DIRECT) {
        const int mode = sink == PART3_AGG_PAIR_DIRECT ? 1 : 0;
        o << "extern \"C\" __global__ __launch_bounds__(kP2AggBlock) void plx_jit_kernel(PartPlan2 pp, AggParams2 ap) {\n"
             "  constexpr Shape csh = JitProg::shape(); constexpr RecLayout2 cl = rec_layout2(JitProg::shape(), " << mode << "u, " << fused::kPackPair << "u);\n"
             "  part2_agg_body<Shape, " << mode << ", p2_agg_chunks_in_flight(cl.rec_words)>(csh, cl, pp, ap);\n}\n}}\n";
        break;
      }
      if (sink >= PART3_SCATTER_PAIR && sink < PART3_AGG_PAIR) {
        const int v = (int)sink - (int)PART3_SCATTER_PAIR, tiles = 1 + (v & 3), hot = (v >> 2) & 1, mode = v >> 3;
        o << "extern \"C\" __global__ __launch_bounds__(kP2MaxBlock) void plx_jit_kernel(Shape dsh, Args args, PartPlan2 pp, ScatterParams2 sp) {\n"
             "  part3_scatter_body<JitProg, " << mode << ", " << tiles << ", " << fused::kPackPair << ", " << (hot ? "true" : "false") << ">(dsh, args, pp, sp);\n}\n}}\n";
        break;
      }
      if (sink >= PART3_AGG && sink != BALLOT && sink != DIRECT_HITS) {
        const int v = (int)sink - (int)PART3_AGG, mode = v & 1, pack = v >> 1;
        o << "extern \"C\" __global__ __launch_bounds__(kP2AggBlock) void plx_jit_kernel(PartPlan2 pp, AggParams2 ap) {\n"
             "  constexpr Shape csh = JitProg::shape(); constexpr RecLayout2 cl = rec_layout2(JitProg::shape(), " << mode << "u, " << pack << "u);\n"
             "  part2_agg_body<Shape, " << mode << ", p2_agg_chunks_in_flight(cl.rec_words)>(csh, cl, pp, ap);\n}\n}}\n";
        break;
      }
      if (sink >= PART3_SCATTER && sink != BALLOT && sink != DIRECT_HITS) {
        const int v = (int)sink - (int)PART3_SCATTER, mode = v & 1, tiles = 1 + ((v >> 1) & 3), pack = (v >> 3) & 3, hot = v >> 5;
        o << "extern \"C\" __global__ __launch_bounds__(kP2MaxBlock) void plx_jit_kernel(Shape dsh, Args args, PartPlan2 pp, ScatterParams2 sp) {\n"
             "  part3_scatter_body<JitProg, " << mode << ", " << tiles << ", " << pack << ", " << (hot ? "true" : "false") << ">(dsh, args, pp, sp);\n}\n}}\n";
        break;
      }
      o << "extern \"C\" __global__ __launch_bounds__(kBlock) void plx_jit_kernel(Shape dsh, Args args, " << sink_type(sink)
        << "::Params sp) {\n  fused_scan_body<JitProg, " << sink_type(sink) << ">(dsh, args, sp);\n}\n}}\n";
      break;
  }
  return o.str();
}

std::atomic<int64_t> g_min_rows{-2};
bool enabled(int64_t n_rows) {
  int64_t m = g_min_rows.load(std::memory_order_relaxed);
  if (m == -2) {
    const char* off = getenv("PLX_JIT");
    const char* e = getenv("PLX_JIT_MIN_ROWS");
    m = (off && off[0] == '0') ? -1 : (e ? (int64_t)atoll(e) : (int64_t)1 << 22);
    g_min_rows.store(m, std::memory_order_relaxed);
  }
  return m >= 0 && n_rows >= m;
}

std::string cache_dir() {
  const char* off = getenv("PLX_JIT_CACHE");
  if (off && off[0] == '0') return "";
  if (const char* d = getenv("PLX_JIT_CACHE_DIR")) return d;
  const char* home = getenv("HOME");
  return home && *home ? std::string(home) + "/.cache/polars_amd/jit" : std::string("/tmp/polars_amd_jit");
}
std::string headers_fingerprint() {
  static const std::string fp = [] {
    uint64_t h = 0xcbf29ce484222325ull;
    for (const char* f : {"fused.hpp", "fused_device.hpp", "fused_sinks.hpp", "fused_shapes.hpp", "partition_device.hpp", "partition2_device.hpp", "partition3_device.hpp", "dev.hpp", "kconfig.hpp", "temporal.hpp", "decimal.hpp"}) {
      if (FILE* fp2 = fopen((include_dir() + "/" + f).c_str(), "rb")) {
        char buf[65536]; size_t n;
        while ((n = fread(buf, 1, sizeof buf, fp2)) > 0) h = fnv1a(std::string(buf, n), h);
        fclose(fp2);
      }
    }
    char out[32]; snprintf(out, sizeof out, "%016llx", (unsigned long long)h);
    return std::string(out);
  }();
  return fp;
}
std::string cache_path(const std::string& src) {
  const std::string dir = cache_dir();
  if (dir.empty()) return "";
  std::string key = src + "|" + headers_fingerprint();
  for (auto& o : compile_options()) if (o.compare(0, 2, "-I") != 0) key += "|" + o;
  char name[64]; snprintf(name, sizeof name, "/%016llx%016llx.hsaco", (unsigned long long)fnv1a(key), (unsigned long long)fnv1a(key, 0x9e3779b97f4a7c15ull));
  return dir + name;
}
bool load_cached(const std::string& path, std::vector<char>* code) {
  if (path.empty()) return false;
  FILE* f = fopen(path.c_str(), "rb");
  if (!f) return false;
  fseek(f, 0, SEEK_END); const long n = ftell(f); fseek(f, 0, SEEK_SET);
  bool ok = n > 0;
  if (ok) { code->resize((size_t)n); ok = fread(code->data(), 1, (size_t)n, f) == (size_t)n; }
  fclose(f);
  return ok;
}
void store_cached(const std::string& path, const std::vector<char>& code) {
  if (path.empty()) return;
  const std::string dir = path.substr(0, path.rfind('/'));
  std::string acc;
  for (size_t i = 1; i <= dir.size(); i++) if (i == dir.size() || dir[i] == '/') { acc = dir.substr(0, i); (void)mkdir(acc.c_str(), 0755); }
  const std::string tmp = path + ".tmp" + std::to_string((long)getpid());
  if (FILE* f = fopen(tmp.c_str(), "wb")) {
    const bool ok = fwrite(code.data(), 1, code.size(), f) == code.size();
    fclose(f);
    if (!ok || rename(tmp.c_str(), path.c_str()) != 0) (void)remove(tmp.c_str());
  }
}
int g_cache_hits = 0;

Entry compile(const Shape& sh, Sink sink) {
  Entry e;
  const auto t0 = std::chrono::steady_clock::now();
  const std::string src = source_for(sh, sink);
  const std::string cpath = cache_path(src);
  {
    std::vector<char> cached;
    if (load_cached(cpath, &cached) && hipModuleLoadData(&e.mod, cached.data()) == hipSuccess && hipModuleGetFunction(&e.fn, e.mod, kernel_symbol(sh, sink).c_str()) == hipSuccess) {
      g_cache_hits++; g_compiled++;
      if (getenv("PLX_JIT_VERBOSE")) fprintf(stderr, "[plx jit] %s: loaded from %s\n", sink_type(sink), cpath.c_str());
      return e;
    }
    (void)hipGetLastError();
    e = Entry{};
  }
  hiprtcProgram prog = nullptr;
  if (hiprtcCreateProgram(&prog, src.c_str(), "plx_jit.hip", 0, nullptr, nullptr) != HIPRTC_SUCCESS) { e.failed = true; return e; }
  const std::vector<std::string> optv = compile_options();
  std::vector<const char*> opts;
  for (auto& x : optv) opts.push_back(x.c_str());
  const hiprtcResult rc = hiprtcCompileProgram(prog, (int)opts.size(), opts.data());
  if (rc != HIPRTC_SUCCESS) {
    size_t n = 0; hiprtcGetProgramLogSize(prog, &n);
    std::string log(n, 0); if (n) hiprtcGetProgramLog(prog, &log[0]);
    set_last_error("jit: hiprtc compile failed: " + log.substr(0, 2000));
    if (getenv("PLX_JIT_VERBOSE")) fprintf(stderr, "[plx jit] compile failed:\n%s\n", log.c_str());
    hiprtcDestroyProgram(&prog);
    e.failed = true;
    return e;
  }
  size_t cs = 0; hiprtcGetCodeSize(prog, &cs);
  std::vector<char> code(cs);
  hiprtcGetCode(prog, code.data());
  hiprtcDestroyProgram(&prog);
  if (hipModuleLoadData(&e.mod, code.data()) != hipSuccess || hipModuleGetFunction(&e.fn, e.mod, kernel_symbol(sh, sink).c_str()) != hipSuccess) { e.failed = true; return e; }
  const double ms = std::chrono::duration<double, std::milli>(std::chrono::steady_clock::now() - t0).count();
  g_compiled++; g_ms += ms;
  if (getenv("PLX_JIT_VERBOSE")) fprintf(stderr, "[plx jit] %s: %.0f ms, %zu bytes\n", sink_type(sink), ms, cs);
  return e;
}
}

std::string selftest(const Shape& sh, Sink sink) {
  const std::string src = source_for(sh, sink);
  hiprtcProgram prog = nullptr;
  if (hiprtcCreateProgram(&prog, src.c_str(), "plx_jit.hip", 0, nullptr, nullptr) != HIPRTC_SUCCESS) return "hiprtcCreateProgram failed";
  const std::vector<std::string> optv = compile_options();
  std::vector<const char*> opts;
  for (auto& x : optv) opts.push_back(x.c_str());
  const hiprtcResult rc = hiprtcCompileProgram(prog, (int)opts.size(), opts.data());
  std::string log;
  if (rc != HIPRTC_SUCCESS) { size_t n = 0; hiprtcGetProgramLogSize(prog, &n); log.assign(n, 0); if (n) hiprtcGetProgramLog(prog, &log[0]); if (log.empty()) log = "hiprtc error"; }
  else if (const char* dir = getenv("PLX_JIT_DUMP_DIR")) {
    size_t cs = 0; hiprtcGetCodeSize(prog, &cs);
    std::vector<char> code(cs);
    hiprtcGetCode(prog, code.data());
    const std::string base = std::string(dir) + "/" + sink_type(sink) + (wide_tiles(sink) ? "_wide" : "") + "_" + std::to_string((int)sink);
    if (FILE* f = fopen((base + ".hsaco").c_str(), "wb")) { fwrite(code.data(), 1, code.size(), f); fclose(f); }
    if (FILE* f = fopen((base + ".hip").c_str(), "wb")) { fwrite(src.data(), 1, src.size(), f); fclose(f); }
  }
  hiprtcDestroyProgram(&prog);
  return log;
}

const char* program_mode(int static_id, int64_t n_rows) { return static_id >= 0 ? "aot" : (enabled(n_rows) ? "jit" : "generic"); }

void set_min_rows(int64_t min_rows) { g_min_rows.store(min_rows < 0 ? -1 : min_rows, std::memory_order_relaxed); }

void stats(int* compiled, double* compile_ms) {
  std::lock_guard<std::mutex> lk(g_mu);
  if (compiled) *compiled = g_compiled;
  if (compile_ms) *compile_ms = g_ms;
}

static hipFunction_t get_fn(const Shape& sh, Sink sink) {
  std::string key((const char*)&sh, sizeof(Shape));
  key.push_back((char)sink);
  std::lock_guard<std::mutex> lk(g_mu);
  auto it = g_cache.find(key);
  if (it == g_cache.end()) it = g_cache.emplace(key, compile(sh, sink)).first;
  return it->second.failed ? nullptr : it->second.fn;
}

bool ensure(const Shape& sh, Sink kind, int64_t n_rows) { return enabled(n_rows) && get_fn(sh, kind) != nullptr; }

bool launch_raw(const Shape& sh, Sink kind, void** kargs, int grid, int block, size_t lds_bytes) {
  hipFunction_t fn = get_fn(sh, kind);
  if (!fn) return false;
  const hipError_t rc = hipModuleLaunchKernel(fn, (unsigned)grid, 1, 1, (unsigned)block, 1, 1, (unsigned)lds_bytes, stream(), kargs, nullptr);
  if (rc != hipSuccess) { set_last_error(std::string("jit: launch failed: ") + hipGetErrorString(rc)); return false; }
  return true;
}

bool launch(const Shape& sh, const Args& args, Sink sink, const void* params, int grid, size_t lds_bytes) {
  if (!enabled(args.n_rows)) return false;
  Shape shc = sh; Args ac = args;
  void* kargs[] = {(void*)&shc, (void*)&ac, const_cast<void*>(params)};
  return launch_raw(sh, sink, kargs, grid, k::kBlock, lds_bytes);
}

}
}
```

polars_amd/csrc/jit.hpp:

```cpp
#pragma once
#include <cstddef>
#include <cstdint>
#include <string>

#include "fused.hpp"

namespace plx {
namespace jit {

enum Sink { REGAGG = 0, LDSAGG, DENSE, HASH, WIDE, JOIN_BUILD, PROBE_AGG, DIRECT_BUILD, DIRECT_PROBE, BITMAP_BUILD,
            PART_COUNT, PART_SCATTER, PART_AGG,
            PART2_SCATTER_HASH, PART2_SCATTER_DIRECT, PART2_AGG_HASH, PART2_AGG_DIRECT,
            PART2_SCATTER_HASH_T2, PART2_SCATTER_DIRECT_T2,
            PART3_SCATTER, PART3_AGG = PART3_SCATTER + 64,
            BALLOT = PART3_AGG + 8,
            DIRECT_HITS,
            PART3_SCATTER_PAIR, PART3_AGG_PAIR = PART3_SCATTER_PAIR + 16, PART3_AGG_PAIR_DIRECT,
            PART3_SCATTER_PAIRV, PART3_AGG_PAIRV = PART3_SCATTER_PAIRV + 8,
            REGAGG_WIDE, LDSAGG_WIDE,
            kNumSinks };
inline Sink part3_scatter_sink(uint32_t mode, uint32_t tiles, uint32_t pack, bool hot) {
  if (pack == fused::kPackPairV) return (Sink)(PART3_SCATTER_PAIRV + (tiles - 1) + (hot ? 4 : 0));
  if (pack == fused::kPackPair) return (Sink)(PART3_SCATTER_PAIR + (tiles - 1) + (hot ? 4 : 0) + 8 * mode);
  return (Sink)(PART3_SCATTER + mode + 2 * (tiles - 1) + 8 * pack + (hot ? 32 : 0));
}
inline Sink part3_agg_sink(uint32_t mode, uint32_t pack) { return pack == fused::kPackPairV ? PART3_AGG_PAIRV : pack == fused::kPackPair ? (Sink)(PART3_AGG_PAIR + mode) : (Sink)(PART3_AGG + mode + 2 * pack); }

bool launch(const fused::Shape& sh, const fused::Args& args, Sink sink, const void* params, int grid, size_t lds_bytes);
bool ensure(const fused::Shape& sh, Sink kind, int64_t n_rows);
bool launch_raw(const fused::Shape& sh, Sink kind, void** kargs, int grid, int block, size_t lds_bytes);
std::string selftest(const fused::Shape& sh, Sink sink);
const char* program_mode(int static_id, int64_t n_rows);
void set_min_rows(int64_t min_rows);
void stats(int* compiled, double* compile_ms);

}
}
```

polars_amd/csrc/kernels_fused.hip:

```cpp
#include "fused_sinks.hpp"
#include "kernels.hpp"
#include "kernels_fused.hpp"
#include "variance.hpp"
#include "scan.hpp"
#include "jit.hpp"
#include <atomic>
#include <cstring>
#include <vector>

#ifdef PLX_HAVE_Q3_SHAPES
#define PLX_STATIC_JOIN_BUILD_CASES \
  case SHAPE_Q3_BUILD: hipLaunchKernelGGL((fused_scan_kernel<StatProg<SHAPE_Q3_BUILD>, JoinBuildSink>), dim3(grid), dim3(kBlock), 0, stream(), sh, args, t); break; \
  case SHAPE_Q3D_BUILD: hipLaunchKernelGGL((fused_scan_kernel<StatProg<SHAPE_Q3D_BUILD>, JoinBuildSink>), dim3(grid), dim3(kBlock), 0, stream(), sh, args, t); break;
#define PLX_STATIC_PROBE_AGG_CASES \
  case SHAPE_Q3_PROBE: hipLaunchKernelGGL((fused_scan_kernel<StatProg<SHAPE_Q3_PROBE>, ProbeAggSink>), dim3(grid), dim3(kBlock), 0, stream(), sh, args, t); break;
#define PLX_STATIC_REGAGG_EXTRA_CASES \
  case SHAPE_Q3_COUNT: launch_static<SHAPE_Q3_COUNT, RegAggSink>(wide, grid, 0, sh, args, sp); break;
#define PLX_STATIC_DIRECT_BUILD_CASES \
  case SHAPE_Q3_BUILD: hipLaunchKernelGGL((fused_scan_kernel<StatProg<SHAPE_Q3_BUILD>, DirectBuildSink>), dim3(grid), dim3(kBlock), 0, stream(), sh, args, t); break; \
  case SHAPE_Q3D_BUILD: hipLaunchKernelGGL((fused_scan_kernel<StatProg<SHAPE_Q3D_BUILD>, DirectBuildSink>), dim3(grid), dim3(kBlock), 0, stream(), sh, args, t); break;
#define PLX_STATIC_DIRECT_PROBE_CASES \
  case SHAPE_Q3_PROBE: hipLaunchKernelGGL((fused_scan_kernel<StatProg<SHAPE_Q3_PROBE>, DirectProbeAggSink>), dim3(grid), dim3(kBlock), 0, stream(), sh, args, t); break;
#ifdef PLX_HAVE_Q3FULL_SHAPES
#define PLX_STATIC_BITMAP_BUILD_CASES \
// ... 13 lines not shown
#else
#define PLX_STATIC_BITMAP_BUILD_CASES
#define PLX_STATIC_Q3F_JOIN_BUILD_CASES
#define PLX_STATIC_Q3F_DIRECT_BUILD_CASES
#define PLX_STATIC_Q3F_REGAGG_CASES
#define PLX_STATIC_DIRECT_BUILD_CASES
#define PLX_STATIC_DIRECT_PROBE_CASES
#define PLX_STATIC_JOIN_BUILD_CASES
#define PLX_STATIC_PROBE_AGG_CASES
#define PLX_STATIC_REGAGG_EXTRA_CASES
#endif

#include <cstdlib>

namespace plx {
namespace k {

static std::string scope_name(const char* aot, const char* other, int static_id) { return static_id >= 0 ? std::string(aot) + "#" + std::to_string(static_id) : std::string(other); }


using namespace dev;
using namespace fused;

__global__ __launch_bounds__(kBlock) void partials_finish_kernel(Shape sh, const unsigned long long* __restrict__ partials, int np, int cells,
                                                                 int cell_stride, unsigned long long* __restrict__ out) {
  __shared__ uint64_t red[kBlock / 64];
  const int cell = blockIdx.x;
  const uint8_t kind = sh.aggs[cell % sh.n_aggs].kind;
  uint64_t x = agg_identity_dev(kind);
  for (int i = threadIdx.x; i < np; i += blockDim.x) x = agg_combine(kind, x, partials[(size_t)i * cell_stride + cell]);
#pragma unroll
  for (int m = 32; m >= 1; m >>= 1) x = agg_combine(kind, x, shfl_xor_u64(x, m));
  if (lane_id() == 0) red[threadIdx.x >> 6] = x;
  __syncthreads();
  if (threadIdx.x == 0) {
    for (int w = 1; w < (int)(blockDim.x >> 6); w++) x = agg_combine(kind, x, red[w]);
    out[cell] = x;
  }
}

static int scan_grid(int64_t n_rows, int blocks_per_cu, const char* knob = nullptr, int tile_rows = kTileRows) {
  if (knob) { const char* e = getenv(knob); const int v = e ? atoi(e) : 0; if (v >= 1 && v <= 32) blocks_per_cu = v; }
  int64_t ntiles = (n_rows + tile_rows - 1) / tile_rows;
  return grid_for(ntiles, kBlock / 64, blocks_per_cu);
}
static_assert(!trust_nullable<StatProg<SHAPE_Q1>, LdsAggSink>() && !trust_nullable<StatProg<SHAPE_CFG2>, RegAggSink>() && !trust_nullable<StatProg<SHAPE_CFG2_NULLX>, RegAggSink>(),
              "rows wider than 16 bytes keep their loads as they were");
static_assert(trust_nullable<StatProg<SHAPE_Q1_ENCODED>, LdsAggSink>() && dict_count(static_shape(SHAPE_Q1_ENCODED)) == 2, "encoded Q1: 15-byte rows, two dictionaries in LDS");
static_assert(trust_nullable<StatProg<SHAPE_Q1_ENCODED_PRICE>, LdsAggSink>() && shape_row_bytes(static_shape(SHAPE_Q1_ENCODED_PRICE)) == 11 && dict_count(static_shape(SHAPE_Q1_ENCODED_PRICE)) == 2,
              "encoded Q1 with the decimal price: 11-byte rows, two dictionaries in LDS");
int64_t scan_waves(int64_t n_rows) { return (int64_t)scan_grid(n_rows, 8) * (kBlock / 64); }
static uint64_t algo_bytes(const Shape& sh, const Args& args) {
  uint64_t algo = 0;
  for (int i = 0; i < sh.n_inputs; i++) algo += (uint64_t)args.n_rows * dtype_width(sh.in_dtype[i]) + (args.in[i].validity ? (uint64_t)args.n_rows / 8 : 0);
  return algo;
}

#define PLX_LAUNCH_SCAN(PROG, SINK, grid, lds, sh, args, sp) \
  hipLaunchKernelGGL((fused_scan_kernel<PROG, SINK>), dim3(grid), dim3(kBlock), (lds), stream(), sh, args, sp)

static bool wide_tiles_knob() {
  static const bool on = [] { const char* e = getenv("PLX_WIDE_TILES"); return !(e && e[0] == '0'); }();
  return on;
}
bool wide_tiles_choice(const Shape& sh, const Args& args, bool compiled, bool knob_on) {
  if (!compiled || !knob_on || args.n_rows < kWideTileRows || !wide_tiles_shape(sh)) return false;
  for (int i = 0; i < sh.n_inputs; i++) {
    if (args.in[i].validity) return false;
    if ((uintptr_t)args.in[i].values % (uintptr_t)(kWideRows * wide_dtype_bytes(sh.in_dtype[i])) != 0) return false;
  }
  return true;
}
static std::atomic<int> g_last_tile_rows{0};
int last_scan_tile_rows() { return g_last_tile_rows.load(std::memory_order_relaxed); }
template <int ID, class Sink>
static void launch_static(bool wide, int grid, size_t lds, const Shape& sh, const Args& args, const typename Sink::Params& sp) {
  if constexpr (wide_tiles_form<StatProg<ID>, Sink>()) {
    if (wide) { hipLaunchKernelGGL((fused_scan_wide_kernel<StatProg<ID>, Sink>), dim3(grid), dim3(kBlock), lds, stream(), sh, args, sp); return; }
  }
  PLX_REQUIRE(!wide, PLX_ERR_INVALID, "fused scan: no wide-tile kernel for this shape");
  PLX_LAUNCH_SCAN(StatProg<ID>, Sink, grid, lds, sh, args, sp);
}

void fused_regagg(const Shape& sh, const Args& args, int static_id, uint64_t* out_host) {
  const bool wide = wide_tiles_choice(sh, args, static_id >= 0 || jit::program_mode(static_id, args.n_rows)[0] == 'j', wide_tiles_knob());
  g_last_tile_rows.store(wide ? kWideTileRows : kTileRows, std::memory_order_relaxed);
  const int grid = scan_grid(args.n_rows, 5, "PLX_BPC_REGAGG", wide ? kWideTileRows : kTileRows);
  Buf partials = dev_alloc(sizeof(uint64_t) * (size_t)(grid + 1) * kMaxAggs);
  unsigned long long* pp = partials->as<unsigned long long>();
  RegAggSink::Params sp{pp};
  {
    ProfileScope ps(scope_name("fused_scan_regagg_static", "fused_scan_regagg_generic", static_id).c_str(), algo_bytes(sh, args), (uint64_t)args.n_rows);
    switch (static_id) {
      case SHAPE_CFG2: launch_static<SHAPE_CFG2, RegAggSink>(wide, grid, 0, sh, args, sp); break;
      case SHAPE_CFG2_NULLX: launch_static<SHAPE_CFG2_NULLX, RegAggSink>(wide, grid, 0, sh, args, sp); break;
      case SHAPE_CFG1: launch_static<SHAPE_CFG1, RegAggSink>(wide, grid, 0, sh, args, sp); break;
      PLX_STATIC_REGAGG_EXTRA_CASES
      PLX_STATIC_Q3F_REGAGG_CASES
      default:
        if (!jit::launch(sh, args, wide ? jit::REGAGG_WIDE : jit::REGAGG, &sp, grid, 0)) {
          g_last_tile_rows.store(kTileRows, std::memory_order_relaxed);
          const DynLaunch d = dyn_launch(sh, args, 0); PLX_LAUNCH_SCAN(DynProg, RegAggSink, grid, d.lds, sh, d.args, sp);
        }
        break;
    }
    PLX_HIP(hipGetLastError());
  }
  unsigned long long* fin = pp + (size_t)grid * kMaxAggs;
  hipLaunchKernelGGL(partials_finish_kernel, dim3(sh.n_aggs), dim3(kBlock), 0, stream(), sh, pp, grid, (int)sh.n_aggs, (int)kMaxAggs, fin);
  PLX_HIP(hipGetLastError());
  d2h_sync(out_host, fin, (size_t)sh.n_aggs * 8);
}

void fused_ballots(const Shape& sh, const Args& args, const BallotOut& out, int static_id) {
  if (args.n_rows == 0) return;
  ProfileScope ps(scope_name("fused_scan_ballots_static", jit::program_mode(-1, args.n_rows)[0] == 'j' ? "fused_scan_ballots[jit]" : "fused_scan_ballots[generic]", static_id).c_str(),
                  algo_bytes(sh, args), (uint64_t)args.n_rows);
  const int grid = scan_grid(args.n_rows, 5, "PLX_BPC_BALLOTS");
  if (!jit::launch(sh, args, jit::BALLOT, &out, grid, 0)) { const DynLaunch d = dyn_launch(sh, args, 0); hipLaunchKernelGGL((fused_scan_kernel<DynProg, BallotSink>), dim3(grid), dim3(kBlock), d.lds, stream(), sh, d.args, out); }
  PLX_HIP(hipGetLastError());
}

void fused_direct_hits(const Shape& sh, const Args& args, const DirectJoinTable& t, const BallotOut& out, int static_id) {
  if (args.n_rows == 0) return;
  ProfileScope ps(scope_name("fused_scan_direct_hits_static", "fused_scan_direct_hits", static_id).c_str(), algo_bytes(sh, args), (uint64_t)args.n_rows);
  const int grid = scan_grid(args.n_rows, 8, "PLX_BPC_DIRECT_HITS");
  DirectHits p{t, out};
  switch (static_id) {
#ifdef PLX_HAVE_Q3_PROBE_SCATTER
    case SHAPE_Q3_PROBE_SCATTER: hipLaunchKernelGGL((fused_scan_kernel<StatProg<SHAPE_Q3_PROBE_SCATTER>, DirectHitsSink>), dim3(grid), dim3(kBlock), 0, stream(), sh, args, p); break;
#endif
    default: if (!jit::launch(sh, args, jit::DIRECT_HITS, &p, grid, 0)) { const DynLaunch d = dyn_launch(sh, args, 0); hipLaunchKernelGGL((fused_scan_kernel<DynProg, DirectHitsSink>), dim3(grid), dim3(kBlock), d.lds, stream(), sh, d.args, p); } break;
  }
  PLX_HIP(hipGetLastError());
}
__global__ __launch_bounds__(kBlock) void direct_slot_rows_kernel(DirectJoinTable t, int64_t n_used, unsigned int* __restrict__ slot_row) {
  for (int64_t o = (int64_t)blockIdx.x * blockDim.x + threadIdx.x; o < n_used; o += (int64_t)gridDim.x * blockDim.x) {
    if ((unsigned int)(o % kOrdChunk) >= t.chunk_used[o / kOrdChunk]) continue;
    const unsigned long long idx = t.ord_key[o] - (unsigned long long)t.kmin;
    slot_row[direct_slot(t, idx, t.bits[idx >> 6])] = t.ord_row[o];
  }
}
void direct_slot_rows(const DirectJoinTable& t, int64_t n_used, uint32_t* slot_row) {
  if (n_used == 0) return;
  ProfileScope ps("direct_slot_rows", (uint64_t)n_used * 28, (uint64_t)n_used);
  hipLaunchKernelGGL(direct_slot_rows_kernel, dim3(grid_for(n_used, kBlock * 4)), dim3(kBlock), 0, stream(), t, n_used, (unsigned int*)slot_row);
  PLX_HIP(hipGetLastError());
}

int lds_agg_copies(int n_groups, int n_aggs) {
  const size_t budget = 60 * 1024;
  int c = 16;
  while (c > 1 && (size_t)n_groups * n_aggs * c * 8 > budget) c >>= 1;
  if ((size_t)n_groups * n_aggs * c * 8 > budget) return 0;
  return c;
}

void fused_lds_agg(const Shape& sh, const Args& args, int n_groups, int static_id, uint64_t* out_dev , unsigned int* oob) {
  const int copies = lds_agg_copies(n_groups, sh.n_aggs);
  PLX_REQUIRE(copies > 0, PLX_ERR_INVALID, "fused_lds_agg: group table does not fit LDS");
  const int cells = n_groups * sh.n_aggs;
  const size_t lds = (size_t)cells * copies * 8;
  const bool wide = wide_tiles_choice(sh, args, static_id >= 0 || jit::program_mode(static_id, args.n_rows)[0] == 'j', wide_tiles_knob());
  g_last_tile_rows.store(wide ? kWideTileRows : kTileRows, std::memory_order_relaxed);
  const int grid = scan_grid(args.n_rows, 5, "PLX_BPC_LDSAGG", wide ? kWideTileRows : kTileRows);
  const bool use_partials = n_groups <= 64;
  Buf partials;
  LdsAggSink::Params sp{};
  sp.n_groups = n_groups; sp.copies = copies; sp.oob = oob;
  if (use_partials) { partials = dev_alloc(sizeof(uint64_t) * (size_t)grid * cells); sp.partials = partials->as<unsigned long long>(); }
  else { init_agg_cells(out_dev, n_groups, sh); sp.global_acc = (unsigned long long*)out_dev; }
  {
    ProfileScope ps(scope_name("fused_scan_ldsagg_static", "fused_scan_ldsagg_generic", static_id).c_str(), algo_bytes(sh, args), (uint64_t)args.n_rows);
    switch (static_id) {
      case SHAPE_Q1: launch_static<SHAPE_Q1, LdsAggSink>(wide, grid, lds, sh, args, sp); break;
      case SHAPE_Q1_ENCODED: launch_static<SHAPE_Q1_ENCODED, LdsAggSink>(wide, grid, lds, sh, args, sp); break;
      case SHAPE_Q1_ENCODED_PRICE: launch_static<SHAPE_Q1_ENCODED_PRICE, LdsAggSink>(wide, grid, lds, sh, args, sp); break;
      default:
        if (!jit::launch(sh, args, wide ? jit::LDSAGG_WIDE : jit::LDSAGG, &sp, grid, lds)) {
          g_last_tile_rows.store(kTileRows, std::memory_order_relaxed);
          const DynLaunch d = dyn_launch(sh, args, lds); PLX_LAUNCH_SCAN(DynProg, LdsAggSink, grid, d.lds, sh, d.args, sp);
        }
        break;
    }
    PLX_HIP(hipGetLastError());
  }
  if (use_partials) {
    hipLaunchKernelGGL(partials_finish_kernel, dim3(cells), dim3(kBlock), 0, stream(), sh, sp.partials, grid, cells, cells, (unsigned long long*)out_dev);
    PLX_HIP(hipGetLastError());
  }
}

__global__ __launch_bounds__(kBlock) void fill_u64_kernel(unsigned long long* p, int64_t n, unsigned long long v) {
  for (int64_t i = (int64_t)blockIdx.x * blockDim.x + threadIdx.x; i < n; i += (int64_t)gridDim.x * blockDim.x) p[i] = v;
}
__global__ __launch_bounds__(kBlock) void init_acc_kernel(unsigned long long* acc, int64_t n_slots, Shape sh) {
  const int64_t total = n_slots * sh.n_aggs;
  for (int64_t i = (int64_t)blockIdx.x * blockDim.x + threadIdx.x; i < total; i += (int64_t)gridDim.x * blockDim.x)
    acc[i] = agg_identity_dev(sh.aggs[i % sh.n_aggs].kind);
}
void fill_u64(uint64_t* p, int64_t n, uint64_t v) {
  if (n == 0) return;
  hipLaunchKernelGGL(fill_u64_kernel, dim3(grid_for(n, kBlock * 4)), dim3(kBlock), 0, stream(), (unsigned long long*)p, n, (unsigned long long)v);
  PLX_HIP(hipGetLastError());
}
void init_agg_cells(uint64_t* acc, int64_t n_slots, const Shape& sh) {
  if (n_slots == 0) return;
  hipLaunchKernelGGL(init_acc_kernel, dim3(grid_for(n_slots * sh.n_aggs, kBlock * 4)), dim3(kBlock), 0, stream(), (unsigned long long*)acc, n_slots, sh);
  PLX_HIP(hipGetLastError());
}

void fused_dense_agg(const Shape& sh, const Args& args, const DenseTable& t, int static_id) {
  if (args.n_rows == 0) return;
  ProfileScope ps("fused_scan_denseagg", algo_bytes(sh, args), (uint64_t)args.n_rows);
  const int grid = scan_grid(args.n_rows, 8);
  switch (static_id) {
    case SHAPE_GB_SUM_CNT_I64: hipLaunchKernelGGL((fused_scan_kernel<StatProg<SHAPE_GB_SUM_CNT_I64>, DenseAggSink>), dim3(grid), dim3(kBlock), 0, stream(), sh, args, t); break;
    case SHAPE_GB_SUM_MEAN_U32_F64: hipLaunchKernelGGL((fused_scan_kernel<StatProg<SHAPE_GB_SUM_MEAN_U32_F64>, DenseAggSink>), dim3(grid), dim3(kBlock), 0, stream(), sh, args, t); break;
    default: if (!jit::launch(sh, args, jit::DENSE, &t, grid, 0)) { const DynLaunch d = dyn_launch(sh, args, 0); hipLaunchKernelGGL((fused_scan_kernel<DynProg, DenseAggSink>), dim3(grid), dim3(kBlock), d.lds, stream(), sh, d.args, t); } break;
  }
  PLX_HIP(hipGetLastError());
}

void fused_hash_agg(const Shape& sh, const Args& args, const HashTable& t, int static_id) {
  if (args.n_rows == 0) return;
  ProfileScope ps("fused_scan_hashagg", algo_bytes(sh, args), (uint64_t)args.n_rows);
  const int grid = scan_grid(args.n_rows, 8);
  switch (static_id) {
    case SHAPE_GB_SUM_CNT_I64: hipLaunchKernelGGL((fused_scan_kernel<StatProg<SHAPE_GB_SUM_CNT_I64>, HashAggSink>), dim3(grid), dim3(kBlock), 0, stream(), sh, args, t); break;
    case SHAPE_GB_SUM_MEAN_U32_F64: hipLaunchKernelGGL((fused_scan_kernel<StatProg<SHAPE_GB_SUM_MEAN_U32_F64>, HashAggSink>), dim3(grid), dim3(kBlock), 0, stream(), sh, args, t); break;
    default: if (!jit::launch(sh, args, jit::HASH, &t, grid, 0)) { const DynLaunch d = dyn_launch(sh, args, 0); hipLaunchKernelGGL((fused_scan_kernel<DynProg, HashAggSink>), dim3(grid), dim3(kBlock), d.lds, stream(), sh, d.args, t); } break;
  }
  PLX_HIP(hipGetLastError());
}



constexpr int kCompactItems = 8;
template <class Occ, class Emit>
__device__ __forceinline__ void compact_slots(int64_t n_slots, unsigned long long* counter, Occ occ, Emit emit) {
  __shared__ uint32_t wave_tot[kBlock / 64];
  __shared__ unsigned long long chunk_base;
  const int lane = lane_id(), wave = threadIdx.x >> 6;
  const int64_t chunk = (int64_t)kBlock * kCompactItems;
  const int64_t nchunks = (n_slots + chunk - 1) / chunk;
  for (int64_t c = blockIdx.x; c < nchunks; c += gridDim.x) {
    const int64_t s0 = c * chunk + threadIdx.x;
    uint32_t bits = 0;
#pragma unroll
    for (int j = 0; j < kCompactItems; j++) { const int64_t s = s0 + (int64_t)j * kBlock; if (s < n_slots && occ(s)) bits |= 1u << j; }
    const uint32_t cnt = (uint32_t)__popc(bits);
    uint32_t incl = cnt;
#pragma unroll
    for (int d = 1; d < 64; d <<= 1) { const uint32_t o = __shfl_up(incl, d, 64); if (lane >= d) incl += o; }
    if (lane == 63) wave_tot[wave] = incl;
    __syncthreads();
    uint32_t wave_off = 0, total = 0;
#pragma unroll
    for (int w = 0; w < kBlock / 64; w++) { if (w < wave) wave_off += wave_tot[w]; total += wave_tot[w]; }
    if (threadIdx.x == 0 && total) chunk_base = atomicAdd(counter, (unsigned long long)total);
    __syncthreads();
    if (total) {
      uint64_t o = chunk_base + wave_off + (incl - cnt);
// ... 565 lines not shown
```

polars_amd/csrc/kernels_fused.hpp:

```cpp
#pragma once
#include <string>
#include <vector>

#include "core.hpp"
#include "fused.hpp"

namespace plx {
namespace k {

void fused_regagg(const fused::Shape& sh, const fused::Args& args, int static_id, uint64_t* out_host);
int lds_agg_copies(int n_groups, int n_aggs);
void fused_lds_agg(const fused::Shape& sh, const fused::Args& args, int n_groups, int static_id, uint64_t* out_dev, unsigned int* oob = nullptr );

bool wide_tiles_choice(const fused::Shape& sh, const fused::Args& args, bool compiled, bool knob_on);
int last_scan_tile_rows();

void fused_dense_agg(const fused::Shape& sh, const fused::Args& args, const fused::DenseTable& t, int static_id);
void fused_hash_agg(const fused::Shape& sh, const fused::Args& args, const fused::HashTable& t, int static_id);
void fused_wide_agg(const fused::Shape& sh, const fused::Args& args, const fused::WideTable& t);
int64_t wide_compact(const fused::WideTable& t, int n_keys, int n_aggs, int64_t out_stride, uint64_t* out_words, uint8_t* out_kvalid, uint64_t* out_acc);
void fused_join_build(const fused::Shape& sh, const fused::Args& args, const fused::JoinAggTable& t, int static_id);
void fused_probe_agg(const fused::Shape& sh, const fused::Args& args, const fused::JoinAggTable& t, int static_id);
int64_t join_agg_compact(const fused::JoinAggTable& t, int n_aggs, int len_idx, uint64_t* out_keys, uint32_t* out_rows, uint64_t* out_acc);
void canonicalise_chains(const fused::JoinAggTable& t, const fused::RepCols& rc, unsigned int max_chain, unsigned int* flags);
int64_t rows_agg_compact(const uint64_t* acc, int64_t n_rows, int n_aggs, int len_idx, uint32_t* out_rows, uint64_t* out_acc);
int64_t chains_agg_compact(const fused::JoinAggTable& t, const fused::Shape& sh, const uint64_t* acc, int len_idx, Buf* out_rows, Buf* out_acc);
int64_t scan_waves(int64_t n_rows);
void fused_ballots(const fused::Shape& sh, const fused::Args& args, const fused::BallotOut& out, int static_id);
void fused_bitmap_build(const fused::Shape& sh, const fused::Args& args, const fused::BitmapBuild& t, int static_id);
void fused_direct_build(const fused::Shape& sh, const fused::Args& args, const fused::DirectJoinTable& t, int static_id);
void fused_direct_probe_agg(const fused::Shape& sh, const fused::Args& args, const fused::DirectJoinTable& t, int static_id);
void fused_direct_hits(const fused::Shape& sh, const fused::Args& args, const fused::DirectJoinTable& t, const fused::BallotOut& out, int static_id);
void direct_slot_rows(const fused::DirectJoinTable& t, int64_t n_used, uint32_t* slot_row);
uint64_t direct_rank(const fused::DirectJoinTable& t, uint32_t* rank_out, int64_t n_used, uint64_t* n_pairs_dev, uint64_t* pairs_out);
int64_t direct_agg_compact(const fused::DirectJoinTable& t, int64_t n_used, int n_aggs, int len_idx, uint64_t* out_keys, uint32_t* out_rows, uint64_t* out_acc);
void fill_u64(uint64_t* p, int64_t n, uint64_t v);
void init_agg_cells(uint64_t* acc, int64_t n_slots, const fused::Shape& sh);
int64_t table_compact(const uint64_t* keys, const uint64_t* acc, int64_t n_slots, int64_t cap, int n_aggs, int occ_agg, uint64_t* out_keys,
                      uint8_t* out_key_valid, uint64_t* out_acc);

void finalize_aggs(const uint64_t* acc, int n_aggs, int64_t G, const fused::FinalSpec& sp, void* out, uint64_t* out_valid);
bool partition_plan(const fused::Shape& sh, double est_groups, bool any_nullable, fused::PartitionPlan* out);
int64_t partitioned_agg(const fused::Shape& sh, const fused::Args& args, const fused::PartitionPlan& pp, int static_id, Buf* out_keys, Buf* out_kvalid,
                        Buf* out_acc, std::string* desc);
struct SrcRange { bool known = false; int64_t mn = 0, mx = 0; bool check = false;  };
bool partition_plan2(const fused::Shape& sh, double est_groups, int packed_bits, int len_idx, int64_t n_rows, int n_hot, fused::PartPlan2* out,
                     const SrcRange* src_ranges = nullptr , const SrcRange* key_range = nullptr );
void select_hot_keys(const fused::HashTable& t, int n_aggs, int len_idx, uint64_t threshold, std::vector<uint64_t>* out, uint64_t* hot_rows = nullptr);
int64_t partitioned_agg2(const fused::Shape& sh, const fused::Args& args, const fused::PartPlan2& pp, int static_id, const std::vector<uint64_t>& hot_keys, Buf* out_keys,
                         Buf* out_kvalid, Buf* out_acc, std::string* desc, int64_t* key_range_out = nullptr, int64_t* wide_stride_out = nullptr);
void touch_filter_set(const int64_t* keys, const uint64_t* validity, int64_t n, unsigned int log2_bits, uint64_t* filter);
bool partitioned_probe_hits(const fused::Shape& sh, const fused::Args& args, const fused::DirectJoinTable& dt, uint64_t n_build, int static_id, ColumnPtr* hits, std::string* desc);
bool partitioned_hash_probe_hits(const fused::Shape& sh, const fused::Args& args, const fused::JoinAggTable& ht, uint64_t n_build, int static_id, ColumnPtr* hits, std::string* desc);
struct JoinCells { Buf key, row; };
bool partitioned_join_build(const fused::Shape& sh, const fused::Args& args, int static_id, const fused::JoinAggTable& t, JoinCells* cells, std::string* desc);
int64_t cells_agg_compact(const JoinCells& cells, const uint64_t* acc, int64_t n_cells, int n_aggs, int len_idx, uint64_t* out_keys, uint32_t* out_rows, uint64_t* out_acc);
double sample_sortedness(const ColumnPtr& c);
bool sample_minmax(const ColumnPtr& c, int64_t* mn, int64_t* mx, int blocks = 64);
void finalize_batch(const uint64_t* acc, int n_aggs, int64_t G, const fused::FinBatch& b);
void decode_key(const uint64_t* packed, const uint8_t* kvalid, int64_t G, const fused::KeyDecode& kd, void* out, uint64_t* out_valid);

}
}
```

Measured before the change: 399.7 billion rows/s.

## Compare dictionary codes directly and narrow integer ops to 32-bit in wide scans

```diff
diff --git a/include/polars_amd.h b/include/polars_amd.h
--- a/include/polars_amd.h
+++ b/include/polars_amd.h
@@ -287,6 +287,13 @@
 int32_t plx_last_scan_tile_rows(void);
 int32_t plx_wide_tiles_choice(int32_t compiled, int32_t knob_on, int64_t n_rows, int32_t n_inputs, const int32_t* dtypes, const int32_t* nullable, const uint64_t* values,
                               const uint64_t* validity);
+int32_t plx_last_scan_narrow(void);
+void plx_set_narrow_codes(int32_t on);
+int32_t plx_narrow_literal(int32_t width, int32_t op, int64_t stride, int64_t base, int64_t literal, int32_t* out);
+int32_t plx_narrow_plan(int32_t n_inputs, const int32_t* dtypes, const int32_t* nullable, int32_t n_ops, const uint8_t* ops, int32_t n_aggs, const uint8_t* aggs, int32_t pred, int32_t key,
+                        int32_t n_keys, const uint8_t* keys, uint32_t* masks);
+int32_t plx_narrow_args(int32_t n_inputs, const int32_t* dtypes, const int32_t* nullable, int32_t n_ops, const uint8_t* ops, int32_t n_aggs, const uint8_t* aggs, int32_t pred, int32_t key,
+                        int32_t n_keys, const uint8_t* keys, const uint64_t* imm, uint64_t* out_imm);
 
 int plx_datagen_lineitem_q1(int64_t n_rows, uint64_t seed, plx_column* out_cols);
 int plx_datagen_lineitem_q1_host(int64_t row0, int64_t n, uint64_t seed, int64_t* shipdate, uint8_t* returnflag, uint8_t* linestatus,
diff --git a/polars_amd/_ffi.py b/polars_amd/_ffi.py
--- a/polars_amd/_ffi.py
+++ b/polars_amd/_ffi.py
@@ -226,6 +226,13 @@
     "plx_last_plan_encodings": (C.c_char_p, []),
     "plx_last_scan_tile_rows": (C.c_int32, []),
     "plx_wide_tiles_choice": (C.c_int32, [C.c_int32, C.c_int32, C.c_int64, C.c_int32, C.POINTER(C.c_int32), C.POINTER(C.c_int32), C.POINTER(C.c_uint64), C.POINTER(C.c_uint64)]),
+    "plx_last_scan_narrow": (C.c_int32, []),
+    "plx_set_narrow_codes": (None, [C.c_int32]),
+    "plx_narrow_literal": (C.c_int32, [C.c_int32, C.c_int32, C.c_int64, C.c_int64, C.c_int64, _i32p]),
+    "plx_narrow_plan": (C.c_int32, [C.c_int32, _i32p, _i32p, C.c_int32, C.POINTER(C.c_uint8), C.c_int32, C.POINTER(C.c_uint8), C.c_int32, C.c_int32, C.c_int32, C.POINTER(C.c_uint8),
+                                    C.POINTER(C.c_uint32)]),
+    "plx_narrow_args": (C.c_int32, [C.c_int32, _i32p, _i32p, C.c_int32, C.POINTER(C.c_uint8), C.c_int32, C.POINTER(C.c_uint8), C.c_int32, C.c_int32, C.c_int32, C.POINTER(C.c_uint8),
+                                    _u64p, _u64p]),
     "plx_profile_enable": (C.c_int, [C.c_int]),
     "plx_profile_fetch": (C.c_int, [C.POINTER(ProfileRecord), C.c_int32, _i32p]),
     "plx_profile_clear": (C.c_int, []),
@@ -301,6 +308,48 @@
                                            (C.c_int32 * n)(*[int(bool(x)) for x in nullable]), (C.c_uint64 * n)(*[int(v) for v in values]), (C.c_uint64 * n)(*[int(v) for v in validity])))
 
 
+def last_scan_narrow() -> bool:
+    return bool(lib().plx_last_scan_narrow())
+
+
+def set_narrow_codes(on) -> None:
+    lib().plx_set_narrow_codes(-1 if on is None else int(bool(on)))
+
+
+def narrow_literal(width: int, op: int, stride: int, base: int, literal: int):
+    out = C.c_int32()
+    return out.value if lib().plx_narrow_literal(int(width), int(op), int(stride), int(base), int(literal), C.byref(out)) == 1 else None
+
+
+def _narrow_program_args(prog):
+    ins, ops, aggs, keys = prog["inputs"], prog["ops"], prog["aggs"], prog.get("keys", [])
+    flat_ops = [int(x) for op in ops for x in op[:5]]
+    flat_aggs = [int(x) for a in aggs for x in a[:2]]
+    return (len(ins), (C.c_int32 * max(1, len(ins)))(*[int(i["dtype"]) for i in ins]), (C.c_int32 * max(1, len(ins)))(*[int(i["nullable"]) for i in ins]), len(ops),
+            (C.c_uint8 * max(1, len(flat_ops)))(*flat_ops), len(aggs), (C.c_uint8 * max(1, len(flat_aggs)))(*flat_aggs), int(prog["pred"]), int(prog["key"]), len(keys),
+            (C.c_uint8 * max(1, len(keys)))(*[int(k) for k in keys]))
+
+
+def narrow_plan(prog) -> dict:
+    masks = (C.c_uint32 * 3)()
+    n = lib().plx_narrow_plan(*_narrow_program_args(prog), masks)
+    if n < 0:
+        raise ValueError("plx_narrow_plan: bad program")
+    bits = lambda m: [pc for pc in range(32) if (m >> pc) & 1]
+    return {"code_cmp": bits(masks[0]), "dead": bits(masks[1]), "narrow32": bits(masks[2]), "n_cmps": n}
+
+
+def narrow_args(prog, imm=None):
+    ops = prog["ops"]
+    imm = [int(op[5]) for op in ops] if imm is None else [int(x) for x in imm]
+    a = (C.c_uint64 * max(1, len(ops)))(*[x & 0xFFFFFFFFFFFFFFFF for x in imm])
+    out = (C.c_uint64 * max(1, len(ops)))()
+    r = lib().plx_narrow_args(*_narrow_program_args(prog), a, out)
+    if r < 0:
+        raise ValueError("plx_narrow_args: bad program")
+    return list(out)[:len(ops)] if r == 1 else None
+
+
 def jit_set_min_rows(min_rows: int) -> None:
     check(lib().plx_jit_set_min_rows(int(min_rows)))
 
diff --git a/polars_amd/csrc/abi.cpp b/polars_amd/csrc/abi.cpp
--- a/polars_amd/csrc/abi.cpp
+++ b/polars_amd/csrc/abi.cpp
@@ -7,6 +7,7 @@
 #include "datagen_device.hpp"
 #include "encoded_inputs.hpp"
 #include "engine.hpp"
+#include "fused_narrow.hpp"
 #include "fused_shapes.hpp"
 #include "jit.hpp"
 #include "join.hpp"
@@ -994,6 +995,45 @@
     args.in[i].values = (const void*)(uintptr_t)values[i]; args.in[i].validity = (const uint64_t*)(uintptr_t)validity[i];
   }
   return k::wide_tiles_choice(sh, args, compiled != 0, knob_on != 0) ? 1 : 0;
+}
+int32_t plx_last_scan_narrow(void) { return k::last_scan_narrow(); }
+void plx_set_narrow_codes(int32_t on) { k::set_narrow_codes(on); }
+int32_t plx_narrow_literal(int32_t width, int32_t op, int64_t stride, int64_t base, int64_t literal, int32_t* out) {
+  int32_t v = 0;
+  if (!out || !fused::narrow_literal(width, op, stride, base, literal, &v)) return 0;
+  *out = v;
+  return 1;
+}
+static bool narrow_shape_from(int32_t n_inputs, const int32_t* dtypes, const int32_t* nullable, int32_t n_ops, const uint8_t* ops, int32_t n_aggs, const uint8_t* aggs, int32_t pred,
+                              int32_t key, int32_t n_keys, const uint8_t* keys, fused::Shape* sh) {
+  if (n_inputs < 0 || n_inputs > fused::kMaxInputs || n_ops < 0 || n_ops > fused::kMaxOps || n_aggs < 0 || n_aggs > fused::kMaxAggs || n_keys < 0 || n_keys > fused::kMaxKeys) return false;
+  if ((n_inputs && (!dtypes || !nullable)) || (n_ops && !ops) || (n_aggs && !aggs) || (n_keys && !keys)) return false;
+  fused::Shape s{};
+  s.n_inputs = (uint8_t)n_inputs; s.n_ops = (uint8_t)n_ops; s.n_aggs = (uint8_t)n_aggs; s.pred = (uint8_t)pred; s.key = (uint8_t)key; s.n_keys = (uint8_t)n_keys;
+  for (int i = 0; i < n_inputs; i++) { s.in_dtype[i] = (uint8_t)dtypes[i]; s.in_nullable[i] = (uint8_t)(nullable[i] != 0); }
+  for (int i = 0; i < n_ops; i++) s.ops[i] = fused::Op{ops[5 * i], ops[5 * i + 1], ops[5 * i + 2], ops[5 * i + 3], ops[5 * i + 4], {0, 0, 0}};
+  for (int i = 0; i < n_aggs; i++) s.aggs[i] = fused::Agg{aggs[2 * i], aggs[2 * i + 1]};
+  for (int i = 0; i < n_keys; i++) s.keys[i] = keys[i];
+  *sh = s;
+  return true;
+}
+int32_t plx_narrow_plan(int32_t n_inputs, const int32_t* dtypes, const int32_t* nullable, int32_t n_ops, const uint8_t* ops, int32_t n_aggs, const uint8_t* aggs, int32_t pred, int32_t key,
+                        int32_t n_keys, const uint8_t* keys, uint32_t* masks) {
+  fused::Shape sh{};
+  if (!masks || !narrow_shape_from(n_inputs, dtypes, nullable, n_ops, ops, n_aggs, aggs, pred, key, n_keys, keys, &sh)) return -1;
+  const fused::NarrowPlan p = fused::narrow_plan(sh);
+  masks[0] = p.code_cmp; masks[1] = p.dead; masks[2] = p.narrow32;
+  return p.n_cmps;
+}
+int32_t plx_narrow_args(int32_t n_inputs, const int32_t* dtypes, const int32_t* nullable, int32_t n_ops, const uint8_t* ops, int32_t n_aggs, const uint8_t* aggs, int32_t pred, int32_t key,
+                        int32_t n_keys, const uint8_t* keys, const uint64_t* imm, uint64_t* out_imm) {
+  fused::Shape sh{};
+  if (!imm || !out_imm || !narrow_shape_from(n_inputs, dtypes, nullable, n_ops, ops, n_aggs, aggs, pred, key, n_keys, keys, &sh)) return -1;
+  fused::Args a{}, o{};
+  for (int i = 0; i < n_ops; i++) a.imm[i] = imm[i];
+  if (!fused::narrow_args(sh, a, &o)) return 0;
+  for (int i = 0; i < n_ops; i++) out_imm[i] = o.imm[i];
+  return 1;
 }
 
 int plx_debug_program_json(const plx_ir* ir, int32_t n_ir, const plx_aexpr* exprs, int32_t n_exprs, int32_t root, char* buf, size_t cap) {
@@ -1104,6 +1144,7 @@
       const bool wide = k::wide_tiles_choice(j.first, aligned, true, true);
       if (j.second == jit::REGAGG && wide) forms.push_back({j.first, jit::REGAGG_WIDE});
       if (j.second == jit::LDSAGG && wide) forms.push_back({j.first, jit::LDSAGG_WIDE});
+      if (j.second == jit::LDSAGG && wide && !fused::narrow_plan_empty(fused::narrow_plan(j.first))) forms.push_back({j.first, jit::LDSAGG_WIDE_NARROW});
     }
     jobs.insert(jobs.end(), forms.begin(), forms.end());
   }
diff --git a/polars_amd/csrc/fused_device.hpp b/polars_amd/csrc/fused_device.hpp
--- a/polars_amd/csrc/fused_device.hpp
+++ b/polars_amd/csrc/fused_device.hpp
@@ -2,6 +2,7 @@
 #include "decimal.hpp"
 #include "dev.hpp"
 #include "fused.hpp"
+#include "fused_narrow.hpp"
 #include "fused_shapes.hpp"
 #include "kconfig.hpp"
 #include "temporal.hpp"
@@ -458,15 +459,29 @@
     default: return (uint64_t)w[2 * e] | ((uint64_t)w[2 * e + 1] << 32);
   }
 }
-template <class P, int ND, class RF>
+template <class P, int ND, bool NARROW = false, class RF>
 __device__ __forceinline__ void run_program_wide(const Args& args, const WideRaw& raw, int j, RF& rf) {
   constexpr Shape sh = P::shape();
+  constexpr NarrowPlan np = NARROW ? narrow_plan(sh) : NarrowPlan{};
 #pragma unroll
   for (int pc = 0; pc < sh.n_ops; pc++) {
     const Op op = sh.ops[pc];
     if (op.code == OP_LOAD) {
 #pragma unroll
       for (int r = 0; r < kRows; r++) rf.set(r, op.dst, wide_unpack(raw.w[op.a], sh.in_dtype[op.a], kRows * j + r));
+      rf.setv(op.dst, (1u << kRows) - 1);
+    } else if (NARROW && ((np.dead >> pc) & 1u)) {
+    } else if (NARROW && ((np.code_cmp >> pc) & 1u)) {
+      const int lit = (int)(uint32_t)args.imm[pc];
+#pragma unroll
+      for (int r = 0; r < kRows; r++) rf.set(r, op.dst, cmp_apply<int>(code_cmp_device_op(op.c), (int)(uint32_t)rf.get(r, op.a), lit) ? 1 : 0);
+      rf.setv(op.dst, (1u << kRows) - 1);
+    } else if (NARROW && ((np.narrow32 >> pc) & 1u)) {
+#pragma unroll
+      for (int r = 0; r < kRows; r++) {
+        const uint32_t a = (uint32_t)rf.get(r, op.a), b = (uint32_t)rf.get(r, op.b);
+        rf.set(r, op.dst, op.code == OP_ADD_I ? (uint64_t)(a + b) : op.code == OP_MUL_I ? (uint64_t)((a & 0xffffffu) * (b & 0xffffffu)) : as_u((double)a));
+      }
       rf.setv(op.dst, (1u << kRows) - 1);
     } else {
       exec_op<true, ND, true>(op, sh, args, pc, 0, rf);
diff --git a/polars_amd/csrc/fused_narrow.hpp b/polars_amd/csrc/fused_narrow.hpp
--- /dev/null
+++ b/polars_amd/csrc/fused_narrow.hpp
@@ -0,0 +1,149 @@
+#pragma once
+#include "fused.hpp"
+
+namespace plx {
+namespace fused {
+
+constexpr int kMaxCodeCmps = 4;
+struct CodeCmp {
+  uint8_t pc;
+  uint8_t slot;
+  uint8_t width;
+  uint8_t op;
+  uint8_t stride_pc, base_pc;
+  uint8_t lit_pc;
+};
+struct NarrowPlan {
+  uint32_t code_cmp, dead, narrow32;
+  uint8_t n_cmps;
+  CodeCmp cmps[kMaxCodeCmps];
+};
+PLX_HD constexpr bool narrow_plan_empty(const NarrowPlan& p) { return (p.code_cmp | p.narrow32) == 0; }
+PLX_HD constexpr int code_cmp_device_op(int op) { return op == 2 ? 3 : op == 4 ? 5 : op; }
+PLX_HD constexpr int narrow_code_bytes(int dtype) { return dtype == 5 ? 1 : dtype == 6 ? 2 : dtype == 7 ? 4 : 0; }
+
+PLX_HD constexpr bool narrow_reads(const Op& op, int slot) { return (op_src_slots(op) >> slot) & 1u; }
+
+PLX_HD constexpr NarrowPlan narrow_plan(const Shape& s) {
+  NarrowPlan p{};
+  uint8_t kind[kSlots] = {}, at[kSlots] = {}, width[kSlots] = {}, stage[kSlots] = {}, stride_pc[kSlots] = {}, base_pc[kSlots] = {}, mul_pc[kSlots] = {}, add_pc[kSlots] = {};
+  bool shared[kSlots] = {};
+  for (int pc = 0; pc < s.n_ops && pc < 32; pc++) {
+    const Op op = s.ops[pc];
+    if (op.code == OP_NOP || op.dst >= kSlots) continue;
+    if (op.code == OP_LOAD) {
+      const int w = op.a < s.n_inputs ? narrow_code_bytes(s.in_dtype[op.a]) : 0;
+      const bool code = (w == 1 || w == 2) && s.in_nullable[op.a] == 0;
+      kind[op.dst] = code ? 1 : 0; at[op.dst] = (uint8_t)pc; width[op.dst] = (uint8_t)w; stage[op.dst] = 0; shared[op.dst] = false;
+      stride_pc[op.dst] = kNone; base_pc[op.dst] = kNone; mul_pc[op.dst] = kNone; add_pc[op.dst] = kNone;
+      continue;
+    }
+    if (op.code == OP_CONST) { kind[op.dst] = 2; at[op.dst] = (uint8_t)pc; continue; }
+    const bool in_place = op.dst == op.a && op.a != op.b && op.a < kSlots && op.b < kSlots && kind[op.a] == 1 && kind[op.b] == 2;
+    if (op.code == OP_MUL_I && in_place && stage[op.a] == 0) { stage[op.a] = 1; stride_pc[op.a] = at[op.b]; mul_pc[op.a] = (uint8_t)pc; continue; }
+    if (op.code == OP_ADD_I && in_place && stage[op.a] <= 1) { stage[op.a] = 2; base_pc[op.a] = at[op.b]; add_pc[op.a] = (uint8_t)pc; continue; }
+    if (op.code == OP_CMP_I && op.a != op.b && op.a < kSlots && op.b < kSlots && kind[op.a] == 1 && kind[op.b] == 2 && !shared[op.a] && p.n_cmps < kMaxCodeCmps) {
+      bool ok = true;
+      if (op.dst != op.a) {
+        bool rewritten = false;
+        for (int q = pc + 1; q < s.n_ops && !rewritten; q++) {
+          if (s.ops[q].code == OP_NOP) continue;
+          if (narrow_reads(s.ops[q], op.a)) ok = false;
+          if (s.ops[q].dst == op.a) rewritten = true;
+        }
+        if (!rewritten) {
+          if (s.pred == op.a || s.key == op.a) ok = false;
+          for (int i = 0; i < s.n_keys; i++) if (s.keys[i] == op.a) ok = false;
+          for (int k = 0; k < s.n_aggs; k++) if (s.aggs[k].src == op.a) ok = false;
+        }
+      }
+      if (ok) {
+        p.cmps[p.n_cmps++] = CodeCmp{(uint8_t)pc, op.a, width[op.a], op.c, stride_pc[op.a], base_pc[op.a], at[op.b]};
+        p.code_cmp |= 1u << pc;
+        if (mul_pc[op.a] != kNone) p.dead |= 1u << mul_pc[op.a];
+        if (add_pc[op.a] != kNone) p.dead |= 1u << add_pc[op.a];
+      }
+    }
+    for (int sl = 0; sl < kSlots; sl++) if (kind[sl] == 1 && narrow_reads(op, sl)) shared[sl] = true;
+    kind[op.dst] = 0;
+  }
+  bool uns[kSlots] = {}, n32[kSlots] = {};
+  for (int pc = 0; pc < s.n_ops && pc < 32; pc++) {
+    const Op op = s.ops[pc];
+    if (op.code == OP_NOP || op.dst >= kSlots || ((p.dead >> pc) & 1u)) continue;
+    bool u = false, n = false;
+    if (op.code == OP_LOAD) u = op.a < s.n_inputs && narrow_code_bytes(s.in_dtype[op.a]) != 0 && s.in_nullable[op.a] == 0;
+    else if (op.code == OP_CONST) u = true;
+    else if ((op.code == OP_ADD_I || op.code == OP_MUL_I) && op.a < kSlots && op.b < kSlots && uns[op.a] && uns[op.b]) { u = true; n = true; p.narrow32 |= 1u << pc; }
+    else if ((op.code == OP_I2F || op.code == OP_U2F) && op.a < kSlots && n32[op.a]) p.narrow32 |= 1u << pc;
+    uns[op.dst] = u; n32[op.dst] = n;
+  }
+  return p;
+}
+
+#ifndef __HIPCC_RTC__
+inline bool narrow_literal(int width, int op, int64_t stride, int64_t base, int64_t lit, int32_t* out) {
+  typedef __int128 i128;
+  if ((width != 1 && width != 2) || op < 0 || op > 5 || stride < 1) return false;
+  const i128 top = (i128)base + (i128)stride * (i128)((1 << (8 * width)) - 1);
+  if (top > (i128)INT64_MAX) return false;
+  const i128 d = (i128)lit - (i128)base, st = (i128)stride;
+  i128 fl = d / st, rem = d % st;
+  if (rem < 0) { fl -= 1; rem += st; }
+  const i128 ce = rem == 0 ? fl : fl + 1;
+  i128 v = 0;
+  switch (op) {
+    case 3: v = fl; break;
+    case 2: v = ce - 1; break;
+    case 5: v = ce; break;
+    case 4: v = fl + 1; break;
+    default: v = rem == 0 ? fl : -1; break;
+  }
+  if (v < -1) v = -1;
+  if (v > 65536) v = 65536;
+  *out = (int32_t)v;
+  return true;
+}
+
+inline bool narrow_args(const Shape& sh, const Args& a, Args* out) {
+  typedef unsigned __int128 u128;
+  const NarrowPlan p = narrow_plan(sh);
+  if (narrow_plan_empty(p)) return false;
+  const u128 lim = (u128)1 << 32, lim24 = (u128)1 << 24;
+  u128 hi[kSlots]; bool known[kSlots];
+  for (int i = 0; i < kSlots; i++) { hi[i] = 0; known[i] = false; }
+  for (int pc = 0; pc < sh.n_ops && pc < 32; pc++) {
+    const Op op = sh.ops[pc];
+    if (op.code == OP_NOP || op.dst >= kSlots || ((p.dead >> pc) & 1u)) continue;
+    if (op.code == OP_LOAD) {
+      const int w = op.a < sh.n_inputs && sh.in_nullable[op.a] == 0 ? narrow_code_bytes(sh.in_dtype[op.a]) : 0;
+      known[op.dst] = w != 0; hi[op.dst] = w ? ((u128)1 << (8 * w)) - 1 : 0;
+    } else if (op.code == OP_CONST) {
+      known[op.dst] = true; hi[op.dst] = (u128)a.imm[pc];
+    } else if ((p.narrow32 >> pc) & 1u) {
+      if (!known[op.a] || hi[op.a] >= lim) return false;
+      if (op.code == OP_ADD_I || op.code == OP_MUL_I) {
+        if (!known[op.b] || hi[op.b] >= lim) return false;
+        if (op.code == OP_MUL_I && (hi[op.a] >= lim24 || hi[op.b] >= lim24)) return false;
+        const u128 r = op.code == OP_ADD_I ? hi[op.a] + hi[op.b] : hi[op.a] * hi[op.b];
+        if (r >= lim) return false;
+        known[op.dst] = true; hi[op.dst] = r;
+      } else known[op.dst] = false;
+    } else known[op.dst] = false;
+  }
+  Args x = a;
+  for (int i = 0; i < p.n_cmps; i++) {
+    const CodeCmp c = p.cmps[i];
+    const int64_t stride = c.stride_pc == kNone ? 1 : (int64_t)a.imm[c.stride_pc], base = c.base_pc == kNone ? 0 : (int64_t)a.imm[c.base_pc];
+    if (c.stride_pc != kNone && a.imm[c.stride_pc] > (uint64_t)INT64_MAX) return false;
+    int32_t lit = 0;
+    if (!narrow_literal(c.width, c.op, stride, base, (int64_t)a.imm[c.lit_pc], &lit)) return false;
+    x.imm[c.pc] = (uint64_t)(int64_t)lit;
+  }
+  *out = x;
+  return true;
+}
+#endif
+
+}
+}
diff --git a/polars_amd/csrc/fused_sinks.hpp b/polars_amd/csrc/fused_sinks.hpp
--- a/polars_amd/csrc/fused_sinks.hpp
+++ b/polars_amd/csrc/fused_sinks.hpp
@@ -97,6 +97,39 @@
       if (p.global_acc) { if (x != agg_identity_dev(kind) || kind == AGG_SUM_F) atomic_agg(kind, p.global_acc + i, x); }
       else p.partials[(size_t)blockIdx.x * cells + i] = x;
     }
+  }
+};
+
+struct LdsAgg16Sink : LdsAggSink {
+  static constexpr int kCopies = 16;
+  bool outside = false;
+  template <class S> __device__ __forceinline__ void init(const S& sh, const Params& p) { outside = false; LdsAggSink::init(sh, p); }
+  template <class S, class RF> __device__ __forceinline__ void consume(const S& sh, const RF& rf, const bool pass[kRows], int64_t row0, const Params& p) {
+    extern __shared__ unsigned long long lds_tbl[];
+    const uint32_t copy = (uint32_t)lane_id() & (uint32_t)(kCopies - 1);
+#pragma unroll
+    for (int r = 0; r < kRows; r++) {
+      const uint64_t gid64 = rf.get(r, sh.key);
+      const bool inside = gid64 < (uint64_t)(uint32_t)p.n_groups;
+      outside = outside || (pass[r] && !inside);
+      if (!(pass[r] && inside)) continue;
+      unsigned long long* cells = lds_tbl + (((uint32_t)gid64 & 0xffffu) * (uint32_t)(sh.n_aggs * kCopies) + copy);
+#pragma unroll
+      for (int k = 0; k < kMaxAggs; k++) {
+        if (k < sh.n_aggs) {
+          const Agg ag = sh.aggs[k];
+          uint64_t v = rf.get(r, ag.src);
+          bool valid = (rf.getv(ag.src) >> r) & 1;
+          if ((ag.kind == AGG_SUM_F || ag.kind == AGG_SUM_I || ag.kind == AGG_COUNT) && !valid) continue;
+          uint64_t x = agg_row_value(ag.kind, v, true, valid, (uint64_t)(row0 + r));
+          lds_atomic_agg(ag.kind, cells + k * kCopies, x);
+        }
+      }
+    }
+  }
+  template <class S> __device__ __forceinline__ void finish(const S& sh, const Params& p) {
+    if (outside && p.oob) *p.oob = 1u;
+    LdsAggSink::finish(sh, p);
   }
 };
 
@@ -503,7 +536,7 @@
 }
 template <class P, class Sink>
 __host__ __device__ constexpr bool trust_nullable() {
-  if constexpr (P::kStatic && (std::is_same<Sink, LdsAggSink>::value || std::is_same<Sink, RegAggSink>::value)) return narrow_rows(P::shape());
+  if constexpr (P::kStatic && (std::is_same<Sink, LdsAggSink>::value || std::is_same<Sink, LdsAgg16Sink>::value || std::is_same<Sink, RegAggSink>::value)) return narrow_rows(P::shape());
   else return false;
 }
 template <class P, class Sink>
@@ -511,7 +544,12 @@
   if constexpr (trust_nullable<P, Sink>()) return wide_tiles_shape(P::shape());
   else return false;
 }
-template <class P, class Sink, bool WIDE = false>
+template <class P, class Sink>
+__host__ __device__ constexpr bool narrow_form() {
+  if constexpr (wide_tiles_form<P, Sink>()) return !narrow_plan_empty(narrow_plan(P::shape()));
+  else return false;
+}
+template <class P, class Sink, bool WIDE = false, bool NARROW = false>
 __device__ __forceinline__ void fused_scan_body(const Shape dsh, const Args args, const typename Sink::Params sp) {
   Sink sink;
   typename RegFileOf<P>::type rf = make_regfile<P>(args);
@@ -533,6 +571,7 @@
     int64_t first_tile = 0;
     if constexpr (WIDE) {
       static_assert(wide_tiles_form<P, Sink>(), "wide tiles: a compiled aggregate scan over narrow rows without nullable inputs");
+      static_assert(!NARROW || narrow_form<P, Sink>(), "narrow form: a wide-tile scan whose plan marks an op");
       const int64_t nwide = args.n_rows / kWideTileRows;
       const int lane = lane_id();
       for (int64_t t = wave; t < nwide; t += nwaves) {
@@ -541,7 +580,7 @@
         wide_load<P>(args, row0, raw);
 #pragma unroll
         for (int j = 0; j < kWideRows / kRows; j++) {
-          run_program_wide<P, ND>(args, raw, j, rf);
+          run_program_wide<P, ND, NARROW>(args, raw, j, rf);
           bool pass[kRows];
 #pragma unroll
           for (int r = 0; r < kRows; r++) pass[r] = sh.pred == kNone || ((rf.get(r, sh.pred) & 1) && ((rf.getv(sh.pred) >> r) & 1));
@@ -574,6 +613,13 @@
 template <class P, class Sink>
 __global__ __launch_bounds__(kBlock) void fused_scan_wide_kernel(Shape dsh, Args args, typename Sink::Params sp) {
   fused_scan_body<P, Sink, true>(dsh, args, sp);
+}
+
+template <class P, class Sink>
+__device__ __forceinline__ void fused_scan_narrow_body(const Shape dsh, const Args args, const typename Sink::Params sp) { fused_scan_body<P, Sink, true, true>(dsh, args, sp); }
+template <class P, class Sink>
+__global__ __launch_bounds__(kBlock) void fused_scan_wide_kernel_narrow(Shape dsh, Args args, typename Sink::Params sp) {
+  fused_scan_narrow_body<P, Sink>(dsh, args, sp);
 }
 
 struct BallotSink {
diff --git a/polars_amd/csrc/jit.cpp b/polars_amd/csrc/jit.cpp
--- a/polars_amd/csrc/jit.cpp
+++ b/polars_amd/csrc/jit.cpp
@@ -32,11 +32,13 @@
 double g_ms = 0;
 
 bool wide_tiles(Sink s) { return s == REGAGG_WIDE || s == LDSAGG_WIDE; }
+bool narrow_form(Sink s) { return s == LDSAGG_WIDE_NARROW; }
 const char* sink_type(Sink s) {
   static const char* n[] = {"RegAggSink", "LdsAggSink", "DenseAggSink", "HashAggSink", "WideAggSink", "JoinBuildSink", "ProbeAggSink", "DirectBuildSink", "DirectProbeAggSink", "BitmapBuildSink",
                             "part_count", "part_scatter", "part_agg", "part2_scatter_hash", "part2_scatter_direct", "part2_agg_hash", "part2_agg_direct", "part2_scatter_hash_t2", "part2_scatter_direct_t2"};
   if (s == REGAGG_WIDE) return "RegAggSink";
   if (s == LDSAGG_WIDE) return "LdsAggSink";
+  if (s == LDSAGG_WIDE_NARROW) return "LdsAgg16Sink";
   if (s == PART3_AGG_PAIRV) return "part3_agg";
   if (s >= PART3_SCATTER_PAIRV && s < PART3_AGG_PAIRV) return "part3_scatter";
   if (s == PART3_AGG_PAIR || s == PART3_AGG_PAIR_DIRECT) return "part3_agg";
@@ -91,7 +93,7 @@
   std::ostringstream o;
   const std::string sym = kernel_symbol(sh, sink);
   o << "#define plx_jit_kernel " << sym << "\n";
-  o << ((sink == BALLOT || sink == DIRECT_HITS || wide_tiles(sink)) ? "#include \"fused_sinks.hpp\"\n" : sink >= PART3_SCATTER ? "#include \"partition3_device.hpp\"\n" : sink >= PART2_SCATTER_HASH ? "#include \"partition2_device.hpp\"\n" : sink >= PART_COUNT ? "#include \"partition_device.hpp\"\n" : "#include \"fused_sinks.hpp\"\n") << "namespace plx { namespace k {\n"
+  o << ((sink == BALLOT || sink == DIRECT_HITS || wide_tiles(sink) || narrow_form(sink)) ? "#include \"fused_sinks.hpp\"\n" : sink >= PART3_SCATTER ? "#include \"partition3_device.hpp\"\n" : sink >= PART2_SCATTER_HASH ? "#include \"partition2_device.hpp\"\n" : sink >= PART_COUNT ? "#include \"partition_device.hpp\"\n" : "#include \"fused_sinks.hpp\"\n") << "namespace plx { namespace k {\n"
        "struct JitProg {\n  static constexpr bool kStatic = true; static constexpr int kId = -2;\n  static constexpr Shape shape() {\n    Shape s{};\n";
   o << "    s.n_inputs = " << (int)sh.n_inputs << "; s.n_ops = " << (int)sh.n_ops << "; s.n_aggs = " << (int)sh.n_aggs << "; s.pred = " << (int)sh.pred
     << "; s.key = " << (int)sh.key << "; s.n_keys = " << (int)sh.n_keys << ";\n";
@@ -125,6 +127,11 @@
            "  part2_agg_body<Shape, " << (sink == PART2_AGG_DIRECT ? 1 : 0) << ", p2_agg_chunks_in_flight(cl.rec_words)>(csh, cl, pp, ap);\n}\n}}\n";
       break;
     default:
+      if (narrow_form(sink)) {
+        o << "extern \"C\" __global__ __launch_bounds__(kBlock) void plx_jit_kernel(Shape dsh, Args args, " << sink_type(sink)
+          << "::Params sp) {\n  fused_scan_narrow_body<JitProg, " << sink_type(sink) << ">(dsh, args, sp);\n}\n}}\n";
+        break;
+      }
       if (wide_tiles(sink)) {
         o << "extern \"C\" __global__ __launch_bounds__(kBlock) void plx_jit_kernel(Shape dsh, Args args, " << sink_type(sink)
           << "::Params sp) {\n  fused_scan_body<JitProg, " << sink_type(sink) << ", true>(dsh, args, sp);\n}\n}}\n";
@@ -197,7 +204,7 @@
 std::string headers_fingerprint() {
   static const std::string fp = [] {
     uint64_t h = 0xcbf29ce484222325ull;
-    for (const char* f : {"fused.hpp", "fused_device.hpp", "fused_sinks.hpp", "fused_shapes.hpp", "partition_device.hpp", "partition2_device.hpp", "partition3_device.hpp", "dev.hpp", "kconfig.hpp", "temporal.hpp", "decimal.hpp"}) {
+    for (const char* f : {"fused.hpp", "fused_narrow.hpp", "fused_device.hpp", "fused_sinks.hpp", "fused_shapes.hpp", "partition_device.hpp", "partition2_device.hpp", "partition3_device.hpp", "dev.hpp", "kconfig.hpp", "temporal.hpp", "decimal.hpp"}) {
       if (FILE* fp2 = fopen((include_dir() + "/" + f).c_str(), "rb")) {
         char buf[65536]; size_t n;
         while ((n = fread(buf, 1, sizeof buf, fp2)) > 0) h = fnv1a(std::string(buf, n), h);
@@ -297,7 +304,7 @@
     size_t cs = 0; hiprtcGetCodeSize(prog, &cs);
     std::vector<char> code(cs);
     hiprtcGetCode(prog, code.data());
-    const std::string base = std::string(dir) + "/" + sink_type(sink) + (wide_tiles(sink) ? "_wide" : "") + "_" + std::to_string((int)sink);
+    const std::string base = std::string(dir) + "/" + sink_type(sink) + (wide_tiles(sink) ? "_wide" : narrow_form(sink) ? "_narrow" : "") + "_" + std::to_string((int)sink);
     if (FILE* f = fopen((base + ".hsaco").c_str(), "wb")) { fwrite(code.data(), 1, code.size(), f); fclose(f); }
     if (FILE* f = fopen((base + ".hip").c_str(), "wb")) { fwrite(src.data(), 1, src.size(), f); fclose(f); }
   }
diff --git a/polars_amd/csrc/jit.hpp b/polars_amd/csrc/jit.hpp
--- a/polars_amd/csrc/jit.hpp
+++ b/polars_amd/csrc/jit.hpp
@@ -18,6 +18,7 @@
             PART3_SCATTER_PAIR, PART3_AGG_PAIR = PART3_SCATTER_PAIR + 16, PART3_AGG_PAIR_DIRECT,
             PART3_SCATTER_PAIRV, PART3_AGG_PAIRV = PART3_SCATTER_PAIRV + 8,
             REGAGG_WIDE, LDSAGG_WIDE,
+            LDSAGG_WIDE_NARROW,
             kNumSinks };
 inline Sink part3_scatter_sink(uint32_t mode, uint32_t tiles, uint32_t pack, bool hot) {
   if (pack == fused::kPackPairV) return (Sink)(PART3_SCATTER_PAIRV + (tiles - 1) + (hot ? 4 : 0));
diff --git a/polars_amd/csrc/kernels_fused.hip b/polars_amd/csrc/kernels_fused.hip
--- a/polars_amd/csrc/kernels_fused.hip
+++ b/polars_amd/csrc/kernels_fused.hip
@@ -119,9 +119,31 @@
   PLX_LAUNCH_SCAN(StatProg<ID>, Sink, grid, lds, sh, args, sp);
 }
 
+static std::atomic<int> g_narrow_pin{-1};
+static std::atomic<int> g_last_narrow{0};
+void set_narrow_codes(int on) { g_narrow_pin.store(on < 0 ? -1 : (on ? 1 : 0), std::memory_order_relaxed); }
+int last_scan_narrow() { return g_last_narrow.load(std::memory_order_relaxed); }
+static bool narrow_codes_knob() {
+  const int pin = g_narrow_pin.load(std::memory_order_relaxed);
+  if (pin >= 0) return pin != 0;
+  const char* e = getenv("PLX_NARROW_CODES");
+  return !(e && e[0] == '0');
+}
+template <int ID>
+static void launch_static_lds(bool wide, const Args* narrow, int grid, size_t lds, const Shape& sh, const Args& args, const LdsAggSink::Params& sp) {
+  if constexpr (narrow_form<StatProg<ID>, LdsAgg16Sink>()) {
+    if (narrow) { hipLaunchKernelGGL((fused_scan_wide_kernel_narrow<StatProg<ID>, LdsAgg16Sink>), dim3(grid), dim3(kBlock), lds, stream(), sh, *narrow, sp); return; }
+  }
+  PLX_REQUIRE(!narrow, PLX_ERR_INVALID, "fused scan: no narrow kernel for this shape");
+  launch_static<ID, LdsAggSink>(wide, grid, lds, sh, args, sp);
+}
+static_assert(narrow_form<StatProg<SHAPE_Q1_ENCODED>, LdsAgg16Sink>() && narrow_form<StatProg<SHAPE_Q1_ENCODED_PRICE>, LdsAgg16Sink>() && !narrow_form<StatProg<SHAPE_Q1>, LdsAgg16Sink>(),
+              "the two encoded Q1 shapes have the narrow form, the plain one has no wide tiles at all");
+
 void fused_regagg(const Shape& sh, const Args& args, int static_id, uint64_t* out_host) {
   const bool wide = wide_tiles_choice(sh, args, static_id >= 0 || jit::program_mode(static_id, args.n_rows)[0] == 'j', wide_tiles_knob());
   g_last_tile_rows.store(wide ? kWideTileRows : kTileRows, std::memory_order_relaxed);
+  g_last_narrow.store(0, std::memory_order_relaxed);
   const int grid = scan_grid(args.n_rows, 5, "PLX_BPC_REGAGG", wide ? kWideTileRows : kTileRows);
   Buf partials = dev_alloc(sizeof(uint64_t) * (size_t)(grid + 1) * kMaxAggs);
   unsigned long long* pp = partials->as<unsigned long long>();
@@ -201,6 +223,9 @@
   const bool wide = wide_tiles_choice(sh, args, static_id >= 0 || jit::program_mode(static_id, args.n_rows)[0] == 'j', wide_tiles_knob());
   g_last_tile_rows.store(wide ? kWideTileRows : kTileRows, std::memory_order_relaxed);
   const int grid = scan_grid(args.n_rows, 5, "PLX_BPC_LDSAGG", wide ? kWideTileRows : kTileRows);
+  Args nargs;
+  const bool narrow = wide && copies == LdsAgg16Sink::kCopies && narrow_codes_knob() && narrow_args(sh, args, &nargs);
+  g_last_narrow.store(narrow ? 1 : 0, std::memory_order_relaxed);
   const bool use_partials = n_groups <= 64;
   Buf partials;
   LdsAggSink::Params sp{};
@@ -211,11 +236,12 @@
     ProfileScope ps(scope_name("fused_scan_ldsagg_static", "fused_scan_ldsagg_generic", static_id).c_str(), algo_bytes(sh, args), (uint64_t)args.n_rows);
     switch (static_id) {
       case SHAPE_Q1: launch_static<SHAPE_Q1, LdsAggSink>(wide, grid, lds, sh, args, sp); break;
-      case SHAPE_Q1_ENCODED: launch_static<SHAPE_Q1_ENCODED, LdsAggSink>(wide, grid, lds, sh, args, sp); break;
-      case SHAPE_Q1_ENCODED_PRICE: launch_static<SHAPE_Q1_ENCODED_PRICE, LdsAggSink>(wide, grid, lds, sh, args, sp); break;
+      case SHAPE_Q1_ENCODED: launch_static_lds<SHAPE_Q1_ENCODED>(wide, narrow ? &nargs : nullptr, grid, lds, sh, args, sp); break;
+      case SHAPE_Q1_ENCODED_PRICE: launch_static_lds<SHAPE_Q1_ENCODED_PRICE>(wide, narrow ? &nargs : nullptr, grid, lds, sh, args, sp); break;
       default:
-        if (!jit::launch(sh, args, wide ? jit::LDSAGG_WIDE : jit::LDSAGG, &sp, grid, lds)) {
+        if (!jit::launch(sh, narrow ? nargs : args, narrow ? jit::LDSAGG_WIDE_NARROW : wide ? jit::LDSAGG_WIDE : jit::LDSAGG, &sp, grid, lds)) {
           g_last_tile_rows.store(kTileRows, std::memory_order_relaxed);
+          g_last_narrow.store(0, std::memory_order_relaxed);
           const DynLaunch d = dyn_launch(sh, args, lds); PLX_LAUNCH_SCAN(DynProg, LdsAggSink, grid, d.lds, sh, d.args, sp);
         }
         break;
diff --git a/polars_amd/csrc/kernels_fused.hpp b/polars_amd/csrc/kernels_fused.hpp
--- a/polars_amd/csrc/kernels_fused.hpp
+++ b/polars_amd/csrc/kernels_fused.hpp
@@ -14,6 +14,8 @@
 
 bool wide_tiles_choice(const fused::Shape& sh, const fused::Args& args, bool compiled, bool knob_on);
 int last_scan_tile_rows();
+int last_scan_narrow();
+void set_narrow_codes(int on);
 
 void fused_dense_agg(const fused::Shape& sh, const fused::Args& args, const fused::DenseTable& t, int static_id);
 void fused_hash_agg(const fused::Shape& sh, const fused::Args& args, const fused::HashTable& t, int static_id);
```

Result: no change. 400.8 billion rows/s (median of 6 runs) (+0.3%).
